# leepaul009/LaneGCN-1

Measured on AMD Instinct MI355X. Metric: Argoverse scenes/sec forward (batch=32, ~10k lane nodes), higher is better.
Workload: dtype f32 (2 fp16 planes per operand, 3 products, fp32 accumulate; range-guarded); 1 GPU; S2: hot path forward (graph_gather+CSR plan+MapNet+A2M+M2M+M2A+A2A), 32 scenes/GPU, 10368 lane nodes, 110592 edges, 1600 actors, random-init weights, inputs resident in HBM, hipGraph replay, 4 forwards in flight on 4 streams; scenes_per_gpu=32, parallelism=dp1 (independent scene shards)

## Files before the change

include/lgcn.h:

```cpp
#ifndef LGCN_H
#define LGCN_H

#include <stdint.h>

#ifdef __cplusplus
extern "C" {
#endif

#define LGCN_VERSION 100
#define LGCN_C 128
#define LGCN_TM 16
#define LGCN_MAX_REL 16

enum {
    LGCN_OK = 0,
    LGCN_EINVAL = -1,
    LGCN_ESHAPE = -2,
    LGCN_EALIGN = -3
};

int lgcn_version(void);
const char *lgcn_strerror(int code);


int lgcn_graph_gather(const int64_t *in, int64_t n_elem,
                      const int64_t *seg_off, const int64_t *seg_base, int n_seg,
                      int64_t *out64, int32_t *out32, void *stream);

int64_t lgcn_csr_rowptr_elems(int64_t n_nodes, int n_rel);
int64_t lgcn_csr_ws_elems(int64_t n_nodes, int n_rel);
int lgcn_csr_build(const int64_t *const *u_host, const int64_t *const *v_host,
                   const int64_t *n_edges_host, int n_rel, int64_t n_nodes,
                   int32_t *rowptr, int32_t *col, int32_t *ws, void *stream);

int64_t lgcn_pairs_ws_elems(int64_t n_agt, int n_scenes);
int lgcn_pairs_build(const float *agt_ctrs, const int32_t *agt_off,
                     const float *ctx_ctrs, const int32_t *ctx_off,
                     int n_scenes, int64_t n_agt, int64_t n_ctx,
                     float dist_th, int legacy_offsets,
                     int32_t *hi, int32_t *wi, int64_t cap,
                     int32_t *n_pairs, int32_t *rowptr, int32_t *ws,
                     void *stream);

typedef struct {
    const float *agt_ctrs; const int32_t *agt_off;
    const float *ctx_ctrs; const int32_t *ctx_off;
    int32_t n_scenes; int32_t legacy_offsets;
    int64_t n_agt, n_ctx;
    float dist_th; int32_t pad_;
    int32_t *hi, *wi; int64_t cap;
    int32_t *n_pairs, *rowptr, *ws;
} lgcn_pairs_job_t;
int lgcn_pairs_build_multi(const lgcn_pairs_job_t *jobs, int n_jobs, void *stream);

typedef struct {
    const int64_t *idx_local; int64_t n_elem;
    const int64_t *seg_off, *seg_base; int32_t n_seg, n_rel;
    int64_t u_off[LGCN_MAX_REL], v_off[LGCN_MAX_REL], n_edges[LGCN_MAX_REL];
    int64_t n_nodes;
    int32_t *rowptr, *col;
    void *cnt;
    int32_t *uv;
    const lgcn_pairs_job_t *jobs; int32_t n_jobs, pad_;
    int32_t *clear_word;
} lgcn_index_t;
int64_t lgcn_index_uv_elems(int64_t n_edges);
int64_t lgcn_index_cnt_words(int64_t n_nodes, int n_rel);
int lgcn_index_build(const lgcn_index_t *p_host, void *stream);


int64_t lgcn_conv_packed_bytes(int cin, int cout, int ks);
int lgcn_conv_pack_weight(const float *w, int cin, int cout, int ks, void *out, void *stream);
int lgcn_conv1d_gn(const float *x, int64_t n_act, int lin, int cin, const void *wp, int cout, int ks, int stride,
                   const float *gamma, const float *beta, float eps, const float *res, int res_mode, int relu,
                   float *out, void *stream);

int lgcn_conv1d_gn_train(const float *x, int64_t n_act, int lin, int cin, const void *wp, int cout, int ks, int stride,
                         const float *gamma, const float *beta, float eps, const float *res, int res_mode, int relu,
                         float *out, float *y, void *stream);

int64_t lgcn_conv_packed_t_bytes(int cin, int cout, int ks);
int lgcn_conv_pack_weight_t(const float *w, int cin, int cout, int ks, void *out, void *stream);
int64_t lgcn_conv1d_gn_bwd_ws_bytes(int64_t n_act, int lin, int cin, int cout, int ks, int stride);
int lgcn_conv1d_gn_bwd(const float *g, const float *x, const float *y, const float *out, int64_t n_act, int lin, int cin,
                       const void *wt, int cout, int ks, int stride, const float *gamma, float eps, int res_mode, int relu,
                       float *dx, float *dw, float *dgamma, float *dbeta, float *dres, void *ws, void *stream);

int lgcn_res1d_gn(const float *x, int64_t n_act, int lin, int cin, int c, int stride, const void *w1p, const float *g1,
                  const float *b1, const void *w2p, const float *g2, const float *b2, const void *wdp, const float *gd,
                  const float *bd, float eps, float *out, void *stream);
int lgcn_res1d_pair_gn(const float *x, int64_t n_act, int lin, int cin, int c, int stride, const void *w1p, const float *g1,
                       const float *b1, const void *w2p, const float *g2, const float *b2, const void *wdp, const float *gd,
                       const float *bd, const void *w1q, const float *g1q, const float *b1q, const void *w2q, const float *g2q,
                       const float *b2q, float eps, float *out, void *stream);


typedef struct lgcn_pred_reg {
    const float *h[8];
    const float *w[8];
    const float *b[8];
    const float *ctrs;
    const float *wd, *bd;
    float *reg, *hd;
    int64_t n_act;
    int32_t n_mod, np2;
} lgcn_pred_reg_t;
int lgcn_pred_reg(const lgcn_pred_reg_t *q, void *stream);

int lgcn_pred_final(const float *f, const float *wc, const float *bc, const float *reg, const float *rot, const float *orig,
                    int64_t n_act, int n_mod, int n_pred, float *cls, float *out, void *stream);

int lgcn_pred_final_train(const float *f, const float *wc, const float *bc, const float *reg, int64_t n_act, int n_mod,
                          int np2, float *cls, float *out, int32_t *order, void *stream);

int64_t lgcn_pred_final_bwd_ws_elems(int64_t n_act);
int lgcn_pred_final_bwd(const float *g_cls, const float *g_out, const int32_t *order, const float *f, const float *wc,
                        int64_t n_act, int n_mod, int np2, float *g_reg, float *d_f, float *d_wc, float *d_bc, float *part,
                        void *stream);

typedef struct lgcn_pred_reg_bwd {
    const float *g_reg;
    const float *g_hd;
    const float *h[8];
    const float *w[8];
    const float *hd, *reg, *ctrs;
    float *d_h[8];
    float *d_w[8];
    float *d_b[8];
    float *d_wd, *d_bd;
    float *part;
    int64_t n_act;
    int32_t n_mod, np2;
} lgcn_pred_reg_bwd_t;
int64_t lgcn_pred_reg_bwd_ws_elems(int64_t n_act, int n_mod, int np2);
int lgcn_pred_reg_bwd(const lgcn_pred_reg_bwd_t *q, void *stream);


int64_t lgcn_scan_ws_elems(int64_t n);
int lgcn_bool_square_bound(const int32_t *rowptr, const int32_t *col, int64_t n, int32_t *cand_ptr, int32_t *ws,
                           void *stream);
int lgcn_bool_square(const int32_t *rowptr, const int32_t *col, int64_t n, const int32_t *cand_ptr, int32_t *cand,
                     int32_t *out_rowptr, int32_t *ws, void *stream);
int lgcn_bool_square_compact(const int32_t *cand_ptr, const int32_t *cand, const int32_t *out_rowptr, int64_t n,
                             int32_t *out_col, int32_t *out_row, void *stream);

int lgcn_cross_edges(const float *ctrs, const float *feats, const int64_t *lane_idcs, int64_t n_nodes, int num_lanes,
                     const int64_t *side_pairs, int64_t n_side, const int64_t *pre_pairs, int64_t n_pre,
                     const int64_t *suc_pairs, int64_t n_suc, float cross_dist, uint8_t *mat, int32_t *partner,
                     void *stream);

int lgcn_widen_i32(const int32_t *in, const int32_t *n_dev, int64_t cap,
// ... 318 lines not shown
```

lanegcn-1_amd/_lib.py:

```python
import ctypes as C
import os

_HERE = os.path.dirname(os.path.abspath(__file__))
LIB_PATH = os.path.join(_HERE, "liblgcn.so")

MAX_REL = 16
REL_IDENT, REL_CSR, REL_RANGE, REL_RANGE16 = 0, 1, 2, 3
F_GN1, F_RELU1, F_GEMM2, F_GN2, F_RES, F_RELU2 = 1, 2, 4, 8, 16, 32
MMA_F32, MMA_BF16X3, MMA_BF16, MMA_F16X2 = 0, 1, 2, 3
MMA_NAMES = {"f32": MMA_F32, "bf16x3": MMA_BF16X3, "bf16": MMA_BF16, "f16x2": MMA_F16X2}


class LgcnError(RuntimeError):
    pass


class Rel(C.Structure):
    _fields_ = [("src", C.c_void_p), ("wp", C.c_void_p), ("mode", C.c_int32), ("ridx", C.c_int32)]


class PairsJob(C.Structure):
    _fields_ = [
        ("agt_ctrs", C.c_void_p), ("agt_off", C.c_void_p), ("ctx_ctrs", C.c_void_p), ("ctx_off", C.c_void_p),
        ("n_scenes", C.c_int32), ("legacy_offsets", C.c_int32), ("n_agt", C.c_int64), ("n_ctx", C.c_int64),
        ("dist_th", C.c_float), ("pad_", C.c_int32),
        ("hi", C.c_void_p), ("wi", C.c_void_p), ("cap", C.c_int64),
        ("n_pairs", C.c_void_p), ("rowptr", C.c_void_p), ("ws", C.c_void_p),
    ]


class Index(C.Structure):
    _fields_ = [
        ("idx_local", C.c_void_p), ("n_elem", C.c_int64),
        ("seg_off", C.c_void_p), ("seg_base", C.c_void_p), ("n_seg", C.c_int32), ("n_rel", C.c_int32),
        ("u_off", C.c_int64 * MAX_REL), ("v_off", C.c_int64 * MAX_REL), ("n_edges", C.c_int64 * MAX_REL),
        ("n_nodes", C.c_int64),
        ("rowptr", C.c_void_p), ("col", C.c_void_p), ("cnt", C.c_void_p), ("uv", C.c_void_p),
        ("jobs", C.c_void_p), ("n_jobs", C.c_int32), ("pad_", C.c_int32),
        ("clear_word", C.c_void_p),
    ]


class PredReg(C.Structure):
    _fields_ = [
        ("h", C.c_void_p * 8), ("w", C.c_void_p * 8), ("b", C.c_void_p * 8),
        ("ctrs", C.c_void_p), ("wd", C.c_void_p), ("bd", C.c_void_p), ("reg", C.c_void_p), ("hd", C.c_void_p),
        ("n_act", C.c_int64), ("n_mod", C.c_int32), ("np2", C.c_int32),
    ]


class PredRegBwd(C.Structure):
    _fields_ = [
        ("g_reg", C.c_void_p), ("g_hd", C.c_void_p), ("h", C.c_void_p * 8), ("w", C.c_void_p * 8),
        ("hd", C.c_void_p), ("reg", C.c_void_p), ("ctrs", C.c_void_p),
        ("d_h", C.c_void_p * 8), ("d_w", C.c_void_p * 8), ("d_b", C.c_void_p * 8),
        ("d_wd", C.c_void_p), ("d_bd", C.c_void_p), ("part", C.c_void_p),
        ("n_act", C.c_int64), ("n_mod", C.c_int32), ("np2", C.c_int32),
    ]


class AttPairsBwd(C.Structure):
    _fields_ = [
        ("agt_ctrs", C.c_void_p), ("ctx_ctrs", C.c_void_p), ("hi", C.c_void_p), ("wi", C.c_void_p), ("n_pairs", C.c_void_p),
        ("cap", C.c_int64),
        ("wd0", C.c_void_p), ("bd0", C.c_void_p), ("wpd2", C.c_void_p), ("gd", C.c_void_p), ("btd", C.c_void_p),
        ("wpc0e", C.c_void_p), ("U", C.c_void_p), ("V", C.c_void_p), ("gc", C.c_void_p), ("btc", C.c_void_p),
        ("wptd2", C.c_void_p), ("wptc0e", C.c_void_p), ("masks", C.c_void_p), ("dS", C.c_void_p),
        ("dc", C.c_void_p), ("d_wd2", C.c_void_p), ("d_wc0e", C.c_void_p), ("d_wd0", C.c_void_p), ("d_bd0", C.c_void_p),
        ("d_gd", C.c_void_p), ("d_btd", C.c_void_p), ("d_gc", C.c_void_p), ("d_btc", C.c_void_p), ("ws", C.c_void_p),
        ("eps", C.c_float), ("n_chunks", C.c_int32),
    ]


class PoolPairsBwd(C.Structure):
    _fields_ = [
        ("ctx_pose", C.c_void_p), ("tgt_pose", C.c_void_p), ("ti", C.c_void_p), ("ci", C.c_void_p), ("n_pairs", C.c_void_p),
        ("cap", C.c_int64),
        ("wp", C.c_void_p), ("bp", C.c_void_p), ("wpc0h", C.c_void_p), ("U", C.c_void_p), ("g", C.c_void_p), ("bt", C.c_void_p),
        ("wptc0h", C.c_void_p), ("masks", C.c_void_p), ("dS", C.c_void_p),
        ("dz", C.c_void_p), ("d_w0h", C.c_void_p), ("d_wp", C.c_void_p), ("d_bp", C.c_void_p), ("d_g", C.c_void_p),
        ("d_bt", C.c_void_p), ("ws", C.c_void_p),
        ("eps", C.c_float), ("n_chunks", C.c_int32),
    ]


class LaneConvBwd(C.Structure):
    _fields_ = [
        ("d_out", C.c_void_p), ("out", C.c_void_p), ("Z", C.c_void_p), ("Y", C.c_void_p), ("T", C.c_void_p), ("X", C.c_void_p),
        ("gamma1", C.c_void_p), ("gamma2", C.c_void_p), ("wpt2", C.c_void_p), ("wpt1", C.c_void_p),
        ("dT", C.c_void_p), ("g2", C.c_void_p), ("dX", C.c_void_p),
        ("d_w2", C.c_void_p), ("d_w1", C.c_void_p), ("d_g2", C.c_void_p), ("d_b2", C.c_void_p), ("d_g1", C.c_void_p),
        ("d_b1", C.c_void_p), ("ws", C.c_void_p),
        ("n_rows", C.c_int64), ("eps", C.c_float), ("n_chunks", C.c_int32), ("ident1", C.c_int32), ("pad_", C.c_int32),
    ]


class RowBlockBwd(C.Structure):
    _fields_ = [
        ("d_out", C.c_void_p), ("out", C.c_void_p), ("pre", C.c_void_p), ("gamma", C.c_void_p),
        ("src", C.c_void_p * 2), ("wpt", C.c_void_p * 2), ("d_src", C.c_void_p * 2), ("d_w", C.c_void_p * 2),
        ("d_res", C.c_void_p), ("d_gamma", C.c_void_p), ("d_beta", C.c_void_p), ("ws", C.c_void_p),
        ("n_rows", C.c_int64), ("ld_w", C.c_int32 * 2), ("eps", C.c_float), ("n_rel", C.c_int32), ("n_chunks", C.c_int32),
        ("pad_", C.c_int32),
    ]


class AggMlp(C.Structure):
    _fields_ = [
        ("n_rows", C.c_int64), ("n_rel", C.c_int32), ("n_rel_csr", C.c_int32),
        ("flags", C.c_int32), ("eps", C.c_float), ("mma", C.c_int32), ("tile_rb", C.c_int32),
        ("rel", Rel * MAX_REL),
        ("rowptr", C.c_void_p), ("col", C.c_void_p),
        ("x4_a", C.c_void_p), ("x4_b", C.c_void_p), ("x4_c", C.c_void_p), ("w4", C.c_void_p),
        ("gn1_g", C.c_void_p), ("gn1_b", C.c_void_p),
        ("wp2", C.c_void_p), ("gn2_g", C.c_void_p), ("gn2_b", C.c_void_p),
        ("res", C.c_void_p), ("out", C.c_void_p), ("out_pre", C.c_void_p),
        ("out_mid", C.c_void_p), ("out_pre2", C.c_void_p),
        ("ch_wq", C.c_void_p), ("ch_gq_g", C.c_void_p), ("ch_gq_b", C.c_void_p), ("ch_wu", C.c_void_p),
        ("ch_u_out", C.c_void_p), ("ch_wv", C.c_void_p), ("ch_v_out", C.c_void_p),
    ]


# ... 30 lines not shown
        ("agent_nodes", C.c_void_p), ("agent_vel", C.c_void_p),
        ("roi_agent", C.c_void_p), ("roi_base", C.c_void_p),
        ("node_mask", C.c_void_p), ("out_feats", C.c_void_p), ("agent_feat", C.c_void_p), ("near", C.c_void_p),
        ("edge_cnt", C.c_void_p),
        ("edge_base", C.c_void_p), ("out_u", C.c_void_p), ("out_v", C.c_void_p), ("a2m_v", C.c_void_p),
    ]


OPT_ADAM, OPT_ADAMW, OPT_SGD = 0, 1, 2
OPT_KINDS = {"adam": OPT_ADAM, "adamw": OPT_ADAMW, "sgd": OPT_SGD}

_P, _I, _L, _F, _D = C.c_void_p, C.c_int, C.c_int64, C.c_float, C.c_double

SIGNATURES = {
    "lgcn_version": (C.c_int, []),
    "lgcn_strerror": (C.c_char_p, [_I]),
    "lgcn_graph_gather": (C.c_int, [_P, _L, _P, _P, _I, _P, _P, _P]),
    "lgcn_csr_rowptr_elems": (C.c_int64, [_L, _I]),
    "lgcn_csr_ws_elems": (C.c_int64, [_L, _I]),
    "lgcn_csr_build": (C.c_int, [_P, _P, _P, _I, _L, _P, _P, _P, _P]),
    "lgcn_pairs_ws_elems": (C.c_int64, [_L, _I]),
    "lgcn_pairs_build": (C.c_int, [_P, _P, _P, _P, _I, _L, _L, _F, _I, _P, _P, _L, _P, _P, _P, _P]),
    "lgcn_pairs_build_multi": (C.c_int, [_P, _I, _P]),
    "lgcn_widen_i32": (C.c_int, [_P, _P, _L, _P, _P]),
    "lgcn_packed_bytes": (C.c_int64, [_I, _I]),
    "lgcn_pack_weight": (C.c_int, [_P, _I, _I, _I, _I, _P, _P]),
    "lgcn_pack_weight_t": (C.c_int, [_P, _I, _I, _P, _P]),
    "lgcn_pack_weight_batch": (C.c_int, [_P, _I, _I, _P]),
    "lgcn_agg_mlp": (C.c_int, [C.POINTER(AggMlp), _P]),
    "lgcn_lc_config": (C.c_int, [_I, _I, C.POINTER(C.c_int32), C.POINTER(C.c_int32)]),
    "lgcn_lc_plan_elems": (C.c_int64, [_L, _I, _I]),
    "lgcn_lc_part_elems": (C.c_int64, [_L, _I, _I]),
    "lgcn_lc_plan_build": (C.c_int, [_P, _P, _L, _I, _I, _I, _I, C.POINTER(C.c_int32), _P, _P]),
    "lgcn_laneconv_fwd": (C.c_int, [C.POINTER(LaneConv), _P]),
    "lgcn_agg_mlp_pair": (C.c_int, [C.POINTER(AggMlp), C.POINTER(AggMlp), _P]),
    "lgcn_agg_mlp_multi": (C.c_int, [C.POINTER(C.POINTER(AggMlp)), _I, _P]),
    "lgcn_gn_bwd": (C.c_int, [_P, _P, _P, _P, _L, _F, _P, _P, _P, _P, _P, _P]),
    "lgcn_gn_fwd": (C.c_int, [_P, _P, _P, _P, _L, _F, _I, _P, _P]),
    "lgcn_gn_cl": (C.c_int, [_P, _L, _I, _I, _P, _P, _F, _P, _I, _I, _I, _P, _P]),
    "lgcn_gn_cl_bwd": (C.c_int, [_P, _P, _P, _P, _L, _I, _I, _F, _P, _P, _P, _P]),
    "lgcn_wgrad": (C.c_int, [C.POINTER(AggMlp), _P, _P, _P, _I, _P]),
    "lgcn_gather_rows": (C.c_int, [_P, _P, _P, _L, _P, _P]),
    "lgcn_gather_sum": (C.c_int, [_P, _P, _P, _L, _P, _P]),
    "lgcn_pair_add": (C.c_int, [_P, _P, _P, _P, _P, _P, _L, _P, _P]),
    "lgcn_check_finite": (C.c_int, [_P, _L, _P, _L, _P, _I, _P]),
    "lgcn_mapnet_input": (C.c_int, [_P, _P, _L] + [_P] * 10 + [_F, _I, _P, _P]),
    "lgcn_att_pairs": (C.c_int, [_P, _P, _P, _P, _P, _L] + [_P] * 10 + [_F, _I, _P, _P]),
    "lgcn_att_pairs_train": (C.c_int, [_P, _P, _P, _P, _P, _L] + [_P] * 10 + [_F, _P, _P, _P]),
    "lgcn_pool_pairs": (C.c_int, [_P, _P, _P, _P, _P, _L] + [_P] * 6 + [_F, _P, _P]),
    "lgcn_pool_pairs_train": (C.c_int, [_P, _P, _P, _P, _P, _L] + [_P] * 6 + [_F, _P, _P, _P]),
    "lgcn_pool_pairs_bwd_ws_elems": (C.c_int64, [_L, _I]),
    "lgcn_pool_pairs_bwd": (C.c_int, [C.POINTER(PoolPairsBwd), _P]),
    "lgcn_att_pairs_bwd_ws_elems": (C.c_int64, [_L, _I]),
    "lgcn_att_pairs_bwd": (C.c_int, [C.POINTER(AttPairsBwd), _P]),
    "lgcn_laneconv_bwd_ws_elems": (C.c_int64, [_L, _I, _I]),
    "lgcn_laneconv_bwd": (C.c_int, [C.POINTER(LaneConvBwd), _P]),
    "lgcn_rowblock_bwd_ws_elems": (C.c_int64, [_L, _I, _I]),
    "lgcn_rowblock_bwd": (C.c_int, [C.POINTER(RowBlockBwd), _P]),
    "lgcn_conv_packed_bytes": (C.c_int64, [_I, _I, _I]),
    "lgcn_conv_pack_weight": (C.c_int, [_P, _I, _I, _I, _P, _P]),
    "lgcn_conv1d_gn": (C.c_int, [_P, _L, _I, _I, _P, _I, _I, _I, _P, _P, _F, _P, _I, _I, _P, _P]),
    "lgcn_conv1d_gn_train": (C.c_int, [_P, _L, _I, _I, _P, _I, _I, _I, _P, _P, _F, _P, _I, _I, _P, _P, _P]),
    "lgcn_conv_packed_t_bytes": (C.c_int64, [_I, _I, _I]),
    "lgcn_conv_pack_weight_t": (C.c_int, [_P, _I, _I, _I, _P, _P]),
    "lgcn_conv1d_gn_bwd_ws_bytes": (C.c_int64, [_L, _I, _I, _I, _I, _I]),
    "lgcn_conv1d_gn_bwd": (C.c_int, [_P, _P, _P, _P, _L, _I, _I, _P, _I, _I, _I, _P, _F, _I, _I, _P, _P, _P, _P, _P, _P, _P]),
    "lgcn_res1d_gn": (C.c_int, [_P, _L, _I, _I, _I, _I, _P, _P, _P, _P, _P, _P, _P, _P, _P, _F, _P, _P]),
    "lgcn_res1d_pair_gn": (C.c_int, [_P, _L, _I, _I, _I, _I, _P, _P, _P, _P, _P, _P, _P, _P, _P, _P, _P, _P, _P, _P, _P, _F, _P, _P]),
    "lgcn_pred_reg": (C.c_int, [C.POINTER(PredReg), _P]),
    "lgcn_pred_final": (C.c_int, [_P, _P, _P, _P, _P, _P, _L, _I, _I, _P, _P, _P]),
    "lgcn_pred_final_train": (C.c_int, [_P, _P, _P, _P, _L, _I, _I, _P, _P, _P, _P]),
    "lgcn_pred_final_bwd_ws_elems": (C.c_int64, [_L]),
    "lgcn_pred_final_bwd": (C.c_int, [_P, _P, _P, _P, _P, _L, _I, _I, _P, _P, _P, _P, _P, _P]),
    "lgcn_pred_reg_bwd_ws_elems": (C.c_int64, [_L, _I, _I]),
    "lgcn_pred_reg_bwd": (C.c_int, [C.POINTER(PredRegBwd), _P]),
    "lgcn_scan_ws_elems": (C.c_int64, [_L]),
    "lgcn_bool_square_bound": (C.c_int, [_P, _P, _L, _P, _P, _P]),
    "lgcn_bool_square": (C.c_int, [_P, _P, _L, _P, _P, _P, _P, _P]),
    "lgcn_bool_square_compact": (C.c_int, [_P, _P, _P, _L, _P, _P, _P]),
    "lgcn_cross_edges": (C.c_int, [_P, _P, _P, _L, _I, _P, _L, _P, _L, _P, _L, _F, _P, _P, _P]),
    "lgcn_index_uv_elems": (C.c_int64, [_L]),
    "lgcn_index_cnt_words": (C.c_int64, [_L, _I]),
    "lgcn_index_build": (C.c_int, [_P, _P]),
    "lgcn_att_pairs_ws": (C.c_int, [_P, _P, _P, _P, _P, _L] + [_P] * 10 + [_F, _I, _I, _P, _P]),
    "lgcn_att_pairs_wi": (C.c_int, [_P, _P, _P, _P, _P, _L] + [_P] * 10 + [_F, _I, _I, _P, _P]),
    "lgcn_pack_weight_kperm": (C.c_int, [_P, _I, _I, _P, _P]),
    "lgcn_pred_loss_fwd": (C.c_int, [_P, _P, _P, _P, _L, _I, _I, _F, _F, _F, _F, _F, _P, _P, _P, _P]),
    "lgcn_pred_loss_bwd": (C.c_int, [_P, _P, _P, _P, _L, _I, _I, _F, _F, _P, _P, _P, _P, _P, _P]),
    "lgcn_conv_packed_f32_bytes": (C.c_int64, [_I, _I, _I]),
    "lgcn_conv_pack_weight_f32": (C.c_int, [_P, _I, _I, _I, _P, _P]),
    "lgcn_conv1d_gn_f32": (C.c_int, [_P, _L, _I, _I, _P, _I, _I, _I, _P, _P, _F, _P, _I, _I, _P, _P, _P]),
    "lgcn_opt_chunk_elems": (C.c_int, []),
    "lgcn_opt_step": (C.c_int, [_P, _I, _P, _I, _I, _D, _D, _D, _D, _D, _D, _I, _D, _D, _I, _F, _F, _P]),
    "lgcn_nms_select": (C.c_int, [_P, _P, _P, _L, _I, _F, _I, _I, _P, _P, _P]),
    "lgcn_goal_decode": (C.c_int, [_P, _P, _P, _L, _P, _P, _L, _P, _P, _P, _P, _P, _I, _I, _F, _P, _P, _P, _P, _P, _P]),
    "lgcn_goal_refine": (C.c_int, [_P, _P, _P, _L, _P, _P]),
    "lgcn_goal_refine_bwd": (C.c_int, [_P, _P, _P, _P, _L, _P, _P, _P, _P]),
    "lgcn_goal_decode_bwd": (C.c_int, [_P, _P, _P, _L, _P, _P, _L, _P, _P, _P, _P, _P, _I, _I, _P, _P, _P, _P, _P, _P, _P]),
    "lgcn_roi_loss_fwd": (C.c_int, [_P, _P, _P, _P, _P, _L, _I, _I, _F, _P, _P, _P, _P, _P]),
    "lgcn_roi_loss_bwd": (C.c_int, [_P, _P, _P, _P, _P, _L, _I, _I, _F, _P, _P, _P, _P, _P, _P, _P, _P]),
    "lgcn_roi_max_lanes": (C.c_int, []),
    "lgcn_roi_max_levels": (C.c_int, []),
    "lgcn_roi_ws_elems": (C.c_int64, [_L, _L, _L, _L, _L]),
    "lgcn_roi_search": (C.c_int, [C.POINTER(Roi), _P]),
    "lgcn_roi_nodes": (C.c_int, [C.POINTER(Roi), _P]),
    "lgcn_roi_edge_count": (C.c_int, [C.POINTER(Roi), _P]),
    "lgcn_roi_edge_fill": (C.c_int, [C.POINTER(Roi), _P]),
}

_lib = None


def load():
    global _lib
    if _lib is not None:
        return _lib
    if not os.path.exists(LIB_PATH):
        raise LgcnError(
            "liblgcn.so not found at %s -- the HIP extension is required (no CPU fallback). "
            "Build it with `python -c 'import __graft_entry__ as g; g.build()'` or "
            "`make -C lanegcn-1_amd/csrc`." % LIB_PATH
        )
    lib = C.CDLL(LIB_PATH)
    for name, (res, args) in SIGNATURES.items():
        fn = getattr(lib, name)
        fn.restype = res
        fn.argtypes = args
    _lib = lib
    return lib


def check(rc, what):
    if rc != 0:
        msg = load().lgcn_strerror(int(rc)).decode()
        raise LgcnError("%s failed: %s (code %d)" % (what, msg, rc))
```

lanegcn-1_amd/csrc/lgcn_index.hip:

```cpp
#include "lgcn_common.hpp"

namespace lgcn {

constexpr int kScanThreads = 256;
constexpr int kScanItems = 8;
constexpr int kScanTile = kScanThreads * kScanItems;

template <int CTRL, int ROW_MASK>
__device__ __forceinline__ int dpp_add_from(int v) {
    return v + __builtin_amdgcn_update_dpp(0, v, CTRL, ROW_MASK, 0xf, false);
}
__device__ __forceinline__ int wave_inclusive_scan(int v, int ) {
    v = dpp_add_from<0x111, 0xf>(v);
    v = dpp_add_from<0x112, 0xf>(v);
    v = dpp_add_from<0x114, 0xf>(v);
    v = dpp_add_from<0x118, 0xf>(v);
    v = dpp_add_from<0x142, 0xa>(v);
    v = dpp_add_from<0x143, 0xc>(v);
    return v;
}

template <int NT>
__device__ __forceinline__ int block_exclusive_scan(int v, int *total, int *lds ) {
    const int lane = threadIdx.x & 63, w = threadIdx.x >> 6;
    const int inc = wave_inclusive_scan(v, lane);
    if (lane == 63) lds[w] = inc;
    __syncthreads();
    if (w == 0) {
        const int t = lane < NT / 64 ? lds[lane] : 0;
        const int run = wave_inclusive_scan(t, lane);
        if (lane < NT / 64) lds[lane] = run - t;
        if (lane == NT / 64 - 1) lds[NT / 64] = run;
    }
    __syncthreads();
    const int base = lds[w];
    *total = lds[NT / 64];
    __syncthreads();
    return base + inc - v;
}

__global__ __launch_bounds__(kScanThreads) void k_scan_blocks(const int32_t *in, int32_t *out,
                                                              int32_t *sums, int64_t n) {
    __shared__ int lds[kScanThreads / 64 + 1];
    const int64_t base = (int64_t)blockIdx.x * kScanTile + (int64_t)threadIdx.x * kScanItems;
    int v[kScanItems];
    int s = 0;
#pragma unroll
    for (int i = 0; i < kScanItems; ++i) {
        v[i] = (base + i < n) ? in[base + i] : 0;
        s += v[i];
    }
    int total;
    int pre = block_exclusive_scan<kScanThreads>(s, &total, lds);
#pragma unroll
    for (int i = 0; i < kScanItems; ++i) {
        if (base + i < n) out[base + i] = pre;
        pre += v[i];
    }
    if (threadIdx.x == 0) sums[blockIdx.x] = total;
}

__global__ __launch_bounds__(1024) void k_scan_sums(int32_t *sums, int nb) {
    __shared__ int lds[1024 / 64 + 1];
    int carry = 0;
    for (int c = 0; c < nb; c += 1024) {
        const int i = c + threadIdx.x;
        const int v = i < nb ? sums[i] : 0;
        int total;
        const int pre = block_exclusive_scan<1024>(v, &total, lds);
        if (i < nb) sums[i] = pre + carry;
        carry += total;
    }
}

__global__ __launch_bounds__(kScanThreads) void k_scan_add_prefix(int32_t *out, const int32_t *sums, int64_t n) {
    __shared__ int lds[kScanThreads / 64 + 1];
    int part = 0;
    for (int i = threadIdx.x; i < (int)blockIdx.x; i += kScanThreads) part += sums[i];
    int add;
    block_exclusive_scan<kScanThreads>(part, &add, lds);
    const int64_t base = (int64_t)blockIdx.x * kScanTile + (int64_t)threadIdx.x * kScanItems;
#pragma unroll
    for (int i = 0; i < kScanItems; ++i)
// ... 170 lines not shown
    __device__ int32_t *wi_base() const { return ws + (n_agt + 1) + n_scenes + 1; }
};
struct PairsJobs { PairsJob j[4]; };

template <int PASS>
__global__ __launch_bounds__(256) void k_pairs_rows(const PairsJobs jobs) {
    const PairsJob &j = jobs.j[blockIdx.y];
    pairs_rows_body<PASS>(j.agt, j.agt_off, j.ctx, j.ctx_off, j.n_scenes, j.n_agt, j.n_ctx, j.th, j.rp(), j.rp(), j.hi_base(),
                          j.wi_base(), j.hi, j.wi, j.cap, j.legacy, j.rowptr_q, (int)blockIdx.x);
}

__device__ __forceinline__ void pairs_scan_bases_body(int32_t *rp, int n_agt, const int32_t *agt_off,
                                                      const int32_t *ctx_off, int n_scenes, int legacy, int64_t cap,
                                                      int32_t *hi_base, int32_t *wi_base, int32_t *n_pairs) {
    __shared__ int lds[1024 / 64 + 1];
    int tot = 0;
    for (int64_t c0 = 0; c0 <= n_agt; c0 += 4096) {
        const int64_t b = c0 + 4 * (int64_t)threadIdx.x;
        int v[4], sum = 0;
#pragma unroll
        for (int k = 0; k < 4; ++k) {
            v[k] = b + k < n_agt ? rp[b + k] : 0;
            sum += v[k];
        }
        int chunk;
        int off = block_exclusive_scan<1024>(sum, &chunk, lds) + tot;
#pragma unroll
        for (int k = 0; k < 4; ++k) {
            if (b + k <= n_agt) rp[b + k] = off;
            off += v[k];
        }
        tot += chunk;
    }
    __syncthreads();
    int carry_h = 0, carry_w = 0;
    for (int c = 0; c < n_scenes; c += 1024) {
        const int i = c + threadIdx.x;
        int th = 0, tw = 0;
        if (i < n_scenes) {
            int a0 = agt_off[i], a1 = agt_off[i + 1];
            a0 = a0 < 0 ? 0 : a0 > n_agt ? n_agt : a0;
            a1 = a1 < a0 ? a0 : a1 > n_agt ? n_agt : a1;
            const bool nonempty = rp[a1] - rp[a0] > 0;
            if (!legacy || nonempty) { th = a1 - a0; tw = ctx_off[i + 1] - ctx_off[i]; }
        }
        int tot_h, tot_w;
        const int ph = block_exclusive_scan<1024>(th, &tot_h, lds);
        const int pw = block_exclusive_scan<1024>(tw, &tot_w, lds);
        if (i < n_scenes) { hi_base[i] = ph + carry_h; wi_base[i] = pw + carry_w; }
        carry_h += tot_h;
        carry_w += tot_w;
    }
    if (threadIdx.x == 0) {
        hi_base[n_scenes] = carry_h;
        *n_pairs = (int64_t)tot > cap ? -tot : tot;
    }
}

__global__ __launch_bounds__(1024) void k_pairs_scan_bases(const PairsJobs jobs) {
    const PairsJob &j = jobs.j[blockIdx.x];
    pairs_scan_bases_body(j.rp(), j.n_agt, j.agt_off, j.ctx_off, j.n_scenes, j.legacy, j.cap, j.hi_base(), j.wi_base(),
                          j.n_pairs);
    if (j.n_agt == 0 && threadIdx.x == 0) j.rowptr_q[0] = 0;
}

constexpr int kIdxScanTile = 4096;
constexpr int kIdxMaxTiles = 1024;

struct IndexParams {
    const int64_t *idx_local, *seg_off, *seg_base;
    int n_seg, n_rel;
    int64_t u_off[LGCN_MAX_REL], v_off[LGCN_MAX_REL];
    int64_t start[LGCN_MAX_REL + 1];
    int64_t n_nodes, n_keys1;
    unsigned long long *cnt;
    int32_t *uv;
    int32_t *rowptr, *col;
    int edge_blocks, scan_blocks, n_jobs;
    int job_blocks[5];
    int32_t *clear_word;
    PairsJobs jobs;
};

__device__ __forceinline__ int64_t to_global(const IndexParams &p, int64_t i) {
    int lo = 0, hi = p.n_seg;
    while (hi - lo > 1) {
        const int mid = (lo + hi) >> 1;
        if (p.seg_off[mid] <= i) lo = mid; else hi = mid;
    }
    return p.idx_local[i] + p.seg_base[lo];
}

template <int PASS>
__global__ __launch_bounds__(256) void k_index_edges(const IndexParams p) {
    __shared__ int s_tile[kIdxMaxTiles];
    const int bid = blockIdx.x;
    if (PASS == 0 && bid == 0 && threadIdx.x == 0 && p.clear_word) *p.clear_word = 0;
    if (bid >= p.edge_blocks) {
        const int b = bid - p.edge_blocks;
        int jn = 0;
        while (jn + 1 < p.n_jobs && b >= p.job_blocks[jn + 1]) ++jn;
        const PairsJob &j = p.jobs.j[jn];
        pairs_rows_body<PASS>(j.agt, j.agt_off, j.ctx, j.ctx_off, j.n_scenes, j.n_agt, j.n_ctx, j.th, j.rp(), j.rp(), j.hi_base(),
                              j.wi_base(), j.hi, j.wi, j.cap, j.legacy, j.rowptr_q, b - p.job_blocks[jn]);
        return;
    }
    if (PASS == 0) {
        for (int i = threadIdx.x; i < p.scan_blocks; i += blockDim.x) s_tile[i] = 0;
        __syncthreads();
    }
    const int64_t total = p.start[p.n_rel];
    for (int64_t e = (int64_t)bid * blockDim.x + threadIdx.x; e < total; e += (int64_t)p.edge_blocks * blockDim.x) {
        int r = 0;
        while (r + 1 < p.n_rel && e >= p.start[r + 1]) ++r;
        if (PASS == 0) {
            const int64_t le = e - p.start[r];
            const int64_t u = to_global(p, p.u_off[r] + le), v = to_global(p, p.v_off[r] + le);
            const bool ok = u >= 0 && u < p.n_nodes && v >= 0 && v < p.n_nodes;
            p.uv[2 * e] = ok ? (int32_t)u : -1;
            p.uv[2 * e + 1] = (int32_t)v;
            if (ok) {
                const int64_t k = csr_key(u, r, p.n_rel);
                atomicAdd(&p.cnt[k], 1ull);
                atomicAdd(&s_tile[k / kIdxScanTile], 1);
            }
        } else {
            const int u = p.uv[2 * e], v = p.uv[2 * e + 1];
            if (u < 0) continue;
            const int64_t k = csr_key(u, r, p.n_rel);
            const unsigned long long a = atomicAdd(&p.cnt[k], 1ull << 32);
            p.col[p.rowptr[k] + (int)(a >> 32)] = v;
        }
    }
    if (PASS == 0) {
        __syncthreads();
        for (int i = threadIdx.x; i < p.scan_blocks; i += blockDim.x)
            if (s_tile[i] != 0) atomicAdd(&p.cnt[p.n_keys1 + i], (unsigned long long)s_tile[i]);
    }
}

__global__ __launch_bounds__(1024) void k_index_scan(const IndexParams p) {
    __shared__ int lds[1024 / 64 + 1];
    const int bid = blockIdx.x;
    if (bid >= p.scan_blocks) {
        const PairsJob &j = p.jobs.j[bid - p.scan_blocks];
        pairs_scan_bases_body(j.rp(), j.n_agt, j.agt_off, j.ctx_off, j.n_scenes, j.legacy, j.cap, j.hi_base(), j.wi_base(),
                              j.n_pairs);
        if (j.n_agt == 0 && threadIdx.x == 0) j.rowptr_q[0] = 0;
        return;
    }
    const int part = (int)threadIdx.x < bid ? (int)p.cnt[p.n_keys1 + threadIdx.x] : 0;
    int before;
    block_exclusive_scan<1024>(part, &before, lds);
    const int64_t b = (int64_t)bid * kIdxScanTile + 4 * (int64_t)threadIdx.x;
    int v[4], sum = 0;
#pragma unroll
    for (int k = 0; k < 4; ++k) {
        v[k] = b + k < p.n_keys1 ? (int)(p.cnt[b + k] & 0xffffffffull) : 0;
        sum += v[k];
    }
    int tile_total;
    int off = block_exclusive_scan<1024>(sum, &tile_total, lds) + before;
#pragma unroll
    for (int k = 0; k < 4; ++k) {
        if (b + k < p.n_keys1) p.rowptr[b + k] = off;
        off += v[k];
    }
}

__global__ __launch_bounds__(256) void k_index_sort(const IndexParams p) {
    const int64_t k = (int64_t)blockIdx.x * blockDim.x + threadIdx.x;
    if (k < kIdxMaxTiles) p.cnt[p.n_keys1 + k] = 0ull;
    if (k >= p.n_keys1) return;
    const unsigned long long w = p.cnt[k];
    if (w == 0ull) return;
    p.cnt[k] = 0ull;
    const int n = (int)(w & 0xffffffffull);
    int32_t *c = p.col + p.rowptr[k];
    for (int i = 1; i < n; ++i) {
        const int x = c[i];
        int q = i - 1;
        while (q >= 0 && c[q] > x) { c[q + 1] = c[q]; --q; }
        c[q + 1] = x;
    }
}

__global__ __launch_bounds__(256) void k_sq_bound(const int32_t *rowptr, const int32_t *col, int64_t n, int32_t *ub) {
    const int64_t u = (int64_t)blockIdx.x * blockDim.x + threadIdx.x;
    if (u > n) return;
    int s = 0;
    if (u < n)
        for (int e = rowptr[u]; e < rowptr[u + 1]; ++e) {
            const int v = col[e];
            if (v >= 0 && v < n) s += rowptr[v + 1] - rowptr[v];
        }
    ub[u] = s;
}

__global__ __launch_bounds__(256) void k_sq_expand(const int32_t *rowptr, const int32_t *col, int64_t n,
                                                   const int32_t *cand_ptr, int32_t *cand, int32_t *cnt) {
    const int64_t u = (int64_t)blockIdx.x * blockDim.x + threadIdx.x;
    if (u > n) return;
    if (u == n) { cnt[n] = 0; return; }
    int32_t *c = cand + cand_ptr[u];
    int k = 0;
    for (int e = rowptr[u]; e < rowptr[u + 1]; ++e) {
        const int v = col[e];
        if (v < 0 || v >= n) continue;
        for (int f = rowptr[v]; f < rowptr[v + 1]; ++f) {
            const int w = col[f];
            int q = k - 1;
            while (q >= 0 && c[q] > w) --q;
            if (q >= 0 && c[q] == w) continue;
            for (int r = k; r > q + 1; --r) c[r] = c[r - 1];
            c[q + 1] = w;
            ++k;
        }
    }
    cnt[u] = k;
}

__global__ __launch_bounds__(256) void k_sq_compact(const int32_t *cand_ptr, const int32_t *cand, const int32_t *out_rowptr,
                                                    int64_t n, int32_t *out_col, int32_t *out_row) {
    const int64_t u = (int64_t)blockIdx.x * blockDim.x + threadIdx.x;
    if (u >= n) return;
    const int b = out_rowptr[u], k = out_rowptr[u + 1] - b;
    const int32_t *c = cand + cand_ptr[u];
    for (int i = 0; i < k; ++i) {
        out_col[b + i] = c[i];
        if (out_row) out_row[b + i] = (int32_t)u;
    }
}

__global__ __launch_bounds__(256) void k_lane_mask(const int64_t *side, int64_t n_side, const int64_t *pre, int64_t n_pre,
                                                   const int64_t *suc, int64_t n_suc, int num_lanes, uint8_t *mat) {
    const int64_t per = n_pre + n_suc + 1;
    const int64_t t = (int64_t)blockIdx.x * blockDim.x + threadIdx.x;
    if (t >= n_side * per) return;
    const int64_t i = t / per, j = t % per;
    const int64_t a = side[2 * i], c = side[2 * i + 1];
    if (a < 0 || a >= num_lanes || c < 0 || c >= num_lanes) return;
    int64_t b = c;
    if (j > 0) {
        const int64_t *pp = j - 1 < n_pre ? pre + 2 * (j - 1) : suc + 2 * (j - 1 - n_pre);
        if (pp[0] != c) return;
        b = pp[1];
        if (b < 0 || b >= num_lanes) return;
    }
    mat[a * num_lanes + b] = 1;
}

__global__ __launch_bounds__(256) void k_cross_edges(const float2 *ctrs, const float2 *feats, const int64_t *lane_idcs,
                                                     int n, const uint8_t *mat, int num_lanes, float cross_dist,
                                                     int32_t *partner) {
    const int lane = threadIdx.x & 63;
    const int h = blockIdx.x * (blockDim.x >> 6) + (threadIdx.x >> 6);
    if (h >= n) return;
    const float2 a = ctrs[h];
    const int64_t la = lane_idcs[h];
    const bool la_ok = la >= 0 && la < num_lanes;
    float best = 3.0e38f;
    int bw = 0x7fffffff;
    for (int w0 = 0; w0 < n; w0 += 64) {
        const int w = w0 + lane;
        if (w < n) {
            const int64_t lb = lane_idcs[w];
            const bool ok = la_ok && lb >= 0 && lb < num_lanes && mat[la * num_lanes + lb] != 0;
// ... 103 lines not shown
        t.v[r] = v_host[r];
        t.start[r + 1] = t.start[r] + n_edges_host[r];
    }
    for (int r = n_rel; r < LGCN_MAX_REL; ++r) { t.u[r] = nullptr; t.v[r] = nullptr; t.start[r + 1] = t.start[n_rel]; }
    const int64_t total = t.start[n_rel];
    if (total > 0x7fffffff || n_nodes > 0x7fffffff) return LGCN_ESHAPE;
    if (total > 0) LGCN_CHECK_PTR(col);
    const int64_t nk1 = lgcn_csr_rowptr_elems(n_nodes, n_rel);
    int32_t *cursor = ws;
    int32_t *sums = ws + nk1;
    hipLaunchKernelGGL(k_zero2, dim3(grid_for(nk1, 256, 1024)), dim3(256), 0, st, rowptr, cursor, nk1);
    if (total > 0) {
        hipLaunchKernelGGL((k_csr_edges<0>), dim3(grid_for(total, 256)), dim3(256), 0, st, t, rowptr, nullptr, nullptr);
    }
    int rc = exclusive_scan(rowptr, rowptr, nk1, sums, st);
    if (rc != LGCN_OK) return rc;
    if (total > 0) {
        hipLaunchKernelGGL((k_csr_edges<1>), dim3(grid_for(total, 256)), dim3(256), 0, st, t, cursor, rowptr, col);
        hipLaunchKernelGGL(k_csr_sort_rows, dim3((unsigned)((nk1 - 1 + 255) / 256)), dim3(256), 0, st,
                           rowptr, col, nk1 - 1);
    }
    return launch_status();
}

int64_t lgcn_pairs_ws_elems(int64_t n_agt, int n_scenes) {
    if (n_agt < 0 || n_scenes < 0) return LGCN_EINVAL;
    return (n_agt + 1) + 2 * (int64_t)n_scenes + 1;
}

static int pairs_job_check(const lgcn_pairs_job_t &q) {
    if (q.n_scenes < 1 || q.n_agt < 0 || q.n_ctx < 0 || q.cap < 0) return LGCN_EINVAL;
    if (q.n_agt > 0x7ffffff0 || q.n_ctx > 0x7ffffff0 || q.cap > 0x7ffffff0) return LGCN_ESHAPE;
    LGCN_CHECK_PTR(q.agt_off); LGCN_CHECK_PTR(q.ctx_off); LGCN_CHECK_PTR(q.n_pairs);
    LGCN_CHECK_PTR(q.rowptr); LGCN_CHECK_PTR(q.ws);
    if (q.n_agt > 0) LGCN_CHECK_PTR(q.agt_ctrs);
    if (q.n_ctx > 0) LGCN_CHECK_PTR(q.ctx_ctrs);
    if (q.cap > 0) { LGCN_CHECK_PTR(q.hi); LGCN_CHECK_PTR(q.wi); }
    return LGCN_OK;
}

int lgcn_pairs_build_multi(const lgcn_pairs_job_t *jobs, int n_jobs, void *stream) {
    if (n_jobs < 1 || n_jobs > 4) return LGCN_EINVAL;
    LGCN_CHECK_PTR(jobs);
    hipStream_t st = (hipStream_t)stream;
    PairsJobs dj;
    int64_t max_rows = 0;
    for (int k = 0; k < n_jobs; ++k) {
        const lgcn_pairs_job_t &q = jobs[k];
        const int rc = pairs_job_check(q);
        if (rc != LGCN_OK) return rc;
        PairsJob &d = dj.j[k];
        d.agt = (const float2 *)q.agt_ctrs; d.agt_off = q.agt_off;
        d.ctx = (const float2 *)q.ctx_ctrs; d.ctx_off = q.ctx_off;
        d.n_scenes = q.n_scenes; d.n_agt = (int)q.n_agt; d.n_ctx = (int)q.n_ctx; d.legacy = q.legacy_offsets; d.th = q.dist_th;
        d.hi = q.hi; d.wi = q.wi; d.cap = q.cap; d.n_pairs = q.n_pairs; d.rowptr_q = q.rowptr; d.ws = q.ws;
        if (q.n_agt > max_rows) max_rows = q.n_agt;
    }
    for (int k = n_jobs; k < 4; ++k) dj.j[k] = dj.j[0];
    const unsigned row_blocks = (unsigned)((max_rows + 3) / 4);
    if (max_rows > 0) hipLaunchKernelGGL((k_pairs_rows<0>), dim3(row_blocks, n_jobs), dim3(256), 0, st, dj);
    hipLaunchKernelGGL(k_pairs_scan_bases, dim3(n_jobs), dim3(1024), 0, st, dj);
    if (max_rows > 0) hipLaunchKernelGGL((k_pairs_rows<1>), dim3(row_blocks, n_jobs), dim3(256), 0, st, dj);
    return launch_status();
}

int lgcn_pairs_build(const float *agt_ctrs, const int32_t *agt_off, const float *ctx_ctrs,
                     const int32_t *ctx_off, int n_scenes, int64_t n_agt, int64_t n_ctx, float dist_th,
                     int legacy_offsets, int32_t *hi, int32_t *wi, int64_t cap, int32_t *n_pairs,
                     int32_t *rowptr, int32_t *ws, void *stream) {
    lgcn_pairs_job_t q;
    q.agt_ctrs = agt_ctrs; q.agt_off = agt_off; q.ctx_ctrs = ctx_ctrs; q.ctx_off = ctx_off;
    q.n_scenes = n_scenes; q.legacy_offsets = legacy_offsets; q.n_agt = n_agt; q.n_ctx = n_ctx;
    q.dist_th = dist_th; q.pad_ = 0; q.hi = hi; q.wi = wi; q.cap = cap; q.n_pairs = n_pairs; q.rowptr = rowptr; q.ws = ws;
    return lgcn_pairs_build_multi(&q, 1, stream);
}

int64_t lgcn_index_uv_elems(int64_t n_edges) { return n_edges < 0 ? (int64_t)LGCN_EINVAL : 2 * n_edges; }

int64_t lgcn_index_cnt_words(int64_t n_nodes, int n_rel) {
    const int64_t k = lgcn_csr_rowptr_elems(n_nodes, n_rel);
    return k < 0 ? k : k + kIdxMaxTiles;
}

int lgcn_index_build(const lgcn_index_t *ph, void *stream) {
    LGCN_CHECK_PTR(ph);
    const lgcn_index_t &q = *ph;
    if (q.n_rel < 1 || q.n_rel > LGCN_MAX_REL || q.n_nodes < 0 || q.n_seg < 1 || q.n_jobs < 0 || q.n_jobs > 4 || q.n_elem < 0)
        return LGCN_EINVAL;
    LGCN_CHECK_PTR(q.rowptr); LGCN_CHECK_PTR(q.cnt);
    if (((uintptr_t)q.cnt & 7u) != 0) return LGCN_EALIGN;
    if (q.n_jobs > 0) LGCN_CHECK_PTR(q.jobs);
    IndexParams p;
    p.idx_local = q.idx_local; p.seg_off = q.seg_off; p.seg_base = q.seg_base; p.n_seg = q.n_seg; p.n_rel = q.n_rel;
    p.start[0] = 0;
    for (int r = 0; r < q.n_rel; ++r) {
        if (q.n_edges[r] < 0 || q.u_off[r] < 0 || q.v_off[r] < 0 || q.u_off[r] + q.n_edges[r] > q.n_elem ||
            q.v_off[r] + q.n_edges[r] > q.n_elem)
            return LGCN_EINVAL;
        p.u_off[r] = q.u_off[r]; p.v_off[r] = q.v_off[r];
        p.start[r + 1] = p.start[r] + q.n_edges[r];
    }
    for (int r = q.n_rel; r < LGCN_MAX_REL; ++r) { p.u_off[r] = p.v_off[r] = 0; p.start[r + 1] = p.start[q.n_rel]; }
    const int64_t total = p.start[q.n_rel];
    if (total > 0x7fffffff || q.n_nodes > 0x7fffffff) return LGCN_ESHAPE;
    const int64_t nk1 = lgcn_csr_rowptr_elems(q.n_nodes, q.n_rel);
    if (nk1 > (int64_t)kIdxScanTile * kIdxMaxTiles) return LGCN_ESHAPE;
    if (total > 0) {
        LGCN_CHECK_PTR(q.idx_local); LGCN_CHECK_PTR(q.seg_off); LGCN_CHECK_PTR(q.seg_base);
        LGCN_CHECK_PTR(q.col); LGCN_CHECK_PTR(q.uv);
    }
    p.n_nodes = q.n_nodes; p.n_keys1 = nk1;
    p.cnt = reinterpret_cast<unsigned long long *>(q.cnt); p.uv = q.uv; p.rowptr = q.rowptr; p.col = q.col;
    p.n_jobs = q.n_jobs;
    p.clear_word = q.clear_word;
    p.job_blocks[0] = 0;
    for (int k = 0; k < 4; ++k) {
        if (k < q.n_jobs) {
            const lgcn_pairs_job_t &jq = q.jobs[k];
            const int rc = pairs_job_check(jq);
            if (rc != LGCN_OK) return rc;
            PairsJob &d = p.jobs.j[k];
            d.agt = (const float2 *)jq.agt_ctrs; d.agt_off = jq.agt_off;
            d.ctx = (const float2 *)jq.ctx_ctrs; d.ctx_off = jq.ctx_off;
            d.n_scenes = jq.n_scenes; d.n_agt = (int)jq.n_agt; d.n_ctx = (int)jq.n_ctx; d.legacy = jq.legacy_offsets; d.th = jq.dist_th;
            d.hi = jq.hi; d.wi = jq.wi; d.cap = jq.cap; d.n_pairs = jq.n_pairs; d.rowptr_q = jq.rowptr; d.ws = jq.ws;
            p.job_blocks[k + 1] = p.job_blocks[k] + (int)((jq.n_agt + 3) / 4);
        } else {
            if (k > 0) p.jobs.j[k] = p.jobs.j[0];
            p.job_blocks[k + 1] = p.job_blocks[k];
        }
    }
    if (q.n_jobs == 0) {
        PairsJob z{};
        for (int k = 0; k < 4; ++k) p.jobs.j[k] = z;
    }
    p.edge_blocks = total > 0 ? (int)grid_for(total, 256, 1024) : 0;
    p.scan_blocks = (int)((nk1 + kIdxScanTile - 1) / kIdxScanTile);
    hipStream_t st = (hipStream_t)stream;
    const unsigned g13 = (unsigned)(p.edge_blocks + p.job_blocks[4]);
    if (g13 > 0) hipLaunchKernelGGL((k_index_edges<0>), dim3(g13), dim3(256), 0, st, p);
    else if (q.clear_word) { hipError_t e = hipMemsetAsync(q.clear_word, 0, 4, st); if (e != hipSuccess) return (int)e; }
    hipLaunchKernelGGL(k_index_scan, dim3((unsigned)(p.scan_blocks + q.n_jobs)), dim3(1024), 0, st, p);
    if (g13 > 0) hipLaunchKernelGGL((k_index_edges<1>), dim3(g13), dim3(256), 0, st, p);
    if (total > 0) hipLaunchKernelGGL(k_index_sort, dim3((unsigned)((nk1 + 255) / 256)), dim3(256), 0, st, p);
    return launch_status();
}

int lgcn_bool_square_bound(const int32_t *rowptr, const int32_t *col, int64_t n, int32_t *cand_ptr, int32_t *ws,
                            void *stream) {
    if (n < 0) return LGCN_EINVAL;
    if (n > 0x7ffffff0) return LGCN_ESHAPE;
    LGCN_CHECK_PTR(rowptr); LGCN_CHECK_PTR(cand_ptr); LGCN_CHECK_PTR(ws);
    hipStream_t st = (hipStream_t)stream;
    hipLaunchKernelGGL(k_sq_bound, dim3(grid_for(n + 1, 256, 1 << 22)), dim3(256), 0, st, rowptr, col, n, cand_ptr);
    return exclusive_scan(cand_ptr, cand_ptr, n + 1, ws, st);
}

int lgcn_bool_square(const int32_t *rowptr, const int32_t *col, int64_t n, const int32_t *cand_ptr, int32_t *cand,
                     int32_t *out_rowptr, int32_t *ws, void *stream) {
    if (n < 0) return LGCN_EINVAL;
    if (n > 0x7ffffff0) return LGCN_ESHAPE;
    LGCN_CHECK_PTR(rowptr); LGCN_CHECK_PTR(cand_ptr); LGCN_CHECK_PTR(out_rowptr); LGCN_CHECK_PTR(ws);
    hipStream_t st = (hipStream_t)stream;
    hipLaunchKernelGGL(k_sq_expand, dim3(grid_for(n + 1, 256, 1 << 22)), dim3(256), 0, st, rowptr, col, n, cand_ptr, cand,
                       out_rowptr);
    return exclusive_scan(out_rowptr, out_rowptr, n + 1, ws, st);
}

int lgcn_bool_square_compact(const int32_t *cand_ptr, const int32_t *cand, const int32_t *out_rowptr, int64_t n,
                             int32_t *out_col, int32_t *out_row, void *stream) {
    if (n < 0) return LGCN_EINVAL;
    if (n == 0) return LGCN_OK;
    LGCN_CHECK_PTR(cand_ptr); LGCN_CHECK_PTR(out_rowptr);
    hipLaunchKernelGGL(k_sq_compact, dim3(grid_for(n, 256, 1 << 22)), dim3(256), 0, (hipStream_t)stream, cand_ptr, cand,
                       out_rowptr, n, out_col, out_row);
    return launch_status();
}

int64_t lgcn_scan_ws_elems(int64_t n) { return n < 0 ? (int64_t)LGCN_EINVAL : scan_ws_elems(n); }

int lgcn_cross_edges(const float *ctrs, const float *feats, const int64_t *lane_idcs, int64_t n_nodes, int num_lanes,
                     const int64_t *side_pairs, int64_t n_side, const int64_t *pre_pairs, int64_t n_pre,
                     const int64_t *suc_pairs, int64_t n_suc, float cross_dist, uint8_t *mat, int32_t *partner,
                     void *stream) {
    if (n_nodes < 0 || num_lanes < 0 || n_side < 0 || n_pre < 0 || n_suc < 0) return LGCN_EINVAL;
    if (n_nodes > 0x7ffffff0 || (int64_t)num_lanes * num_lanes > 0x7ffffff0) return LGCN_ESHAPE;
    if (n_nodes == 0) return LGCN_OK;
    LGCN_CHECK_PTR(ctrs); LGCN_CHECK_PTR(feats); LGCN_CHECK_PTR(lane_idcs); LGCN_CHECK_PTR(partner);
    if (num_lanes > 0) LGCN_CHECK_PTR(mat);
    if (n_side > 0) LGCN_CHECK_PTR(side_pairs);
    if (n_pre > 0) LGCN_CHECK_PTR(pre_pairs);
    if (n_suc > 0) LGCN_CHECK_PTR(suc_pairs);
    hipStream_t st = (hipStream_t)stream;
    if (num_lanes > 0) {
        hipError_t e = hipMemsetAsync(mat, 0, (size_t)num_lanes * num_lanes, st);
        if (e != hipSuccess) return (int)e;
    }
    const int64_t work = n_side * (n_pre + n_suc + 1);
    if (work > 0)
        hipLaunchKernelGGL(k_lane_mask, dim3(grid_for(work, 256, 1 << 22)), dim3(256), 0, st, side_pairs, n_side, pre_pairs,
                           n_pre, suc_pairs, n_suc, num_lanes, mat);
    hipLaunchKernelGGL(k_cross_edges, dim3((unsigned)((n_nodes + 3) / 4)), dim3(256), 0, st, (const float2 *)ctrs,
                       (const float2 *)feats, lane_idcs, (int)n_nodes, mat, num_lanes, cross_dist, partner);
    return launch_status();
}

int lgcn_widen_i32(const int32_t *in, const int32_t *n_dev, int64_t cap, int64_t *out, void *stream) {
    if (cap < 0) return LGCN_EINVAL;
    if (cap == 0) return LGCN_OK;
    LGCN_CHECK_PTR(in); LGCN_CHECK_PTR(n_dev); LGCN_CHECK_PTR(out);
    hipLaunchKernelGGL(k_widen, dim3(grid_for(cap, 256, 1024)), dim3(256), 0, (hipStream_t)stream, in, n_dev, cap, out);
    return launch_status();
}

}
```

lanegcn-1_amd/csrc/lgcn_mma_bf.hpp:

```cpp
#pragma once
#include "lgcn_common.hpp"
#include "lgcn_tile.hpp"

namespace lgcn {

typedef __bf16 bf16x8 __attribute__((ext_vector_type(8)));
typedef __bf16 bf16x2 __attribute__((ext_vector_type(2)));
typedef _Float16 f16x8 __attribute__((ext_vector_type(8)));
typedef _Float16 f16x2 __attribute__((ext_vector_type(2)));
typedef float f32x2 __attribute__((ext_vector_type(2)));
typedef float f32x4 __attribute__((ext_vector_type(4)));

constexpr int kLDB = kC + 8;

template <int F> struct Fmt;
template <> struct Fmt<0> {
    static constexpr int NP = 3, NPROD = 6;
    static constexpr int PA[6] = {2, 0, 1, 1, 0, 0}, PB[6] = {0, 2, 1, 0, 1, 0};
    static __device__ __forceinline__ uint32_t pack(float a, float b) {
        const f32x2 v = {a, b};
        return __builtin_bit_cast(uint32_t, __builtin_convertvector(v, bf16x2));
    }
    static __device__ __forceinline__ f32x2 unpack(uint32_t u) {
        return f32x2{__builtin_bit_cast(float, u << 16), __builtin_bit_cast(float, u & 0xffff0000u)};
// ... 127 lines not shown
__device__ __forceinline__ void gemm_pass(const uint16_t *__restrict__ A, const uint4 *__restrict__ Bw,
                                          const uint4 *__restrict__ Bw_next, BPair<F> &r, int wave, int lane,
                                          f32x4 (&acc)[RB][2]) {
    const uint16_t *arow = A + (lane & 15) * kLDB + 8 * (lane >> 4);
    load_b<F>(r.b[1], Bw, wave, lane, 1);
    kstep<RB, F>(arow, 0, r.b[0], acc);
    load_b<F>(r.b[0], Bw, wave, lane, 2);
    kstep<RB, F>(arow, 1, r.b[1], acc);
    load_b<F>(r.b[1], Bw, wave, lane, 3);
    kstep<RB, F>(arow, 2, r.b[0], acc);
    if (Bw_next != nullptr) load_b<F>(r.b[0], Bw_next, wave, lane, 0);
    kstep<RB, F>(arow, 3, r.b[1], acc);
}

template <int F>
__device__ __forceinline__ void gemm2_prefetch(BPair<F> &r, const uint4 *__restrict__ Bw, int wave, int lane) {
    load_b<F>(r.b[1], Bw, wave, lane, 1);
}
template <int F>
__device__ __forceinline__ void gemm2_prefetch(BOne<F> &, const uint4 *__restrict__, int, int) {}
template <int RB, int F>
__device__ __forceinline__ void gemm2_pass(const uint16_t *__restrict__ A, const uint4 *__restrict__ Bw, BOne<F> &r,
                                           int wave, int lane, f32x4 (&acc)[RB][2]) {
    gemm_pass<RB, F>(A, Bw, nullptr, r, wave, lane, acc);
}
template <int RB, int F>
__device__ __forceinline__ void gemm2_pass(const uint16_t *__restrict__ A, const uint4 *__restrict__ Bw, BPair<F> &r,
                                           int wave, int lane, f32x4 (&acc)[RB][2]) {
    const uint16_t *arow = A + (lane & 15) * kLDB + 8 * (lane >> 4);
    kstep<RB, F>(arow, 0, r.b[0], acc);
    load_b<F>(r.b[0], Bw, wave, lane, 2);
    kstep<RB, F>(arow, 1, r.b[1], acc);
    load_b<F>(r.b[1], Bw, wave, lane, 3);
    kstep<RB, F>(arow, 2, r.b[0], acc);
    kstep<RB, F>(arow, 3, r.b[1], acc);
}

template <int RB>
__device__ __forceinline__ void acc_store(float *T, const f32x4 (&acc)[RB][2], int lane, int wave) {
#pragma unroll
    for (int rb = 0; rb < RB; ++rb)
#pragma unroll
        for (int cb = 0; cb < 2; ++cb) {
            float *p = T + (16 * rb + 4 * (lane >> 4)) * kLDA + 32 * wave + 16 * cb + (lane & 15);
#pragma unroll
            for (int i = 0; i < 4; ++i) p[i * kLDA] = acc[rb][cb][i];
        }
}

template <int RB>
__device__ __forceinline__ void acc_zero(f32x4 (&acc)[RB][2]) {
#pragma unroll
    for (int rb = 0; rb < RB; ++rb)
#pragma unroll
        for (int cb = 0; cb < 2; ++cb) acc[rb][cb] = f32x4{0.f, 0.f, 0.f, 0.f};
}

template <int F>
__device__ __forceinline__ void row_split_store(uint16_t *planes, int plane_elems, int row, int t, const RowVals &r) {
#pragma unroll
    for (int j = 0; j < 4; ++j) split_store<F>(planes, plane_elems, row, 4 * (t & 7) + 32 * j, r.v[j]);
}

template <int F>
__device__ __forceinline__ void lin2_relu_split(uint16_t *planes, int plane_elems, int row, int t, float x, float y,
                                                const float *__restrict__ w1, const float *__restrict__ b1) {
    const int c0 = 4 * (t & 7);
#pragma unroll
    for (int j = 0; j < 4; ++j) {
        const int c = c0 + 32 * j;
        const float4 wa = *reinterpret_cast<const float4 *>(w1 + 2 * c);
        const float4 wb = *reinterpret_cast<const float4 *>(w1 + 2 * c + 4);
        const float4 bb = *reinterpret_cast<const float4 *>(b1 + c);
        float4 o;
        o.x = relu_nan(x * wa.x + y * wa.y + bb.x);
        o.y = relu_nan(x * wa.z + y * wa.w + bb.y);
        o.z = relu_nan(x * wb.x + y * wb.y + bb.z);
        o.w = relu_nan(x * wb.z + y * wb.w + bb.w);
        split_store<F>(planes, plane_elems, row, c, o);
    }
}


}
```

lanegcn-1_amd/csrc/lgcn_rowmlp_bf.hip:

```cpp
#include "lgcn_common.hpp"
#include "lgcn_tile.hpp"
#include "lgcn_mma_bf.hpp"
#include <type_traits>

namespace lgcn {

constexpr int LGCN_RB_ONE = 3;

template <int F>
__device__ __forceinline__ void pack_block_bf(const float *__restrict__ W, int ld, uint16_t *__restrict__ out, int transpose,
                                              int i) {
    if (i >= 4 * 4 * 2 * 64) return;
    const int lane = i & 63, cb = (i >> 6) & 1, s = (i >> 7) & 3, w = i >> 9;
    const int orow = 32 * w + 16 * cb + (lane & 15), k0 = 32 * s + 8 * (lane >> 4);
    float v[8];
#pragma unroll
    for (int j = 0; j < 8; ++j) v[j] = transpose ? W[(int64_t)(k0 + j) * ld + orow] : W[(int64_t)orow * ld + k0 + j];
#pragma unroll
    for (int p = 0; p < Fmt<F>::NP; ++p) {
        uint32_t q[4];
#pragma unroll
        for (int j = 0; j < 4; ++j) {
            q[j] = Fmt<F>::pack(v[2 * j], v[2 * j + 1]);
            const f32x2 r = Fmt<F>::unpack(q[j]);
// ... 376 lines not shown
        }
        lds_barrier();
        if (my_live) row_store_global(p.ch_u_out + my_n * kC, my_rt, row_load(T + (upper ? 32 : 0) * kLDA, my_rt));
    };
    if (two && upper) gemm2_prefetch<F>(bfrag, reinterpret_cast<const uint4 *>(p.wp2), wave, lane);
    if (my_has_row) {
        {
            const float *rbase = (flags & LGCN_F_RES) ? p.res : p.out;
            const float *rp_ = rbase + (my_live ? my_n : 0) * kC + 4 * (my_rt & 7);
#pragma unroll
            for (int j = 0; j < 4; ++j) resv.v[j] = *reinterpret_cast<const float4 *>(rp_ + 32 * j);
        }
        RowVals r = row_load(T + (upper ? 32 : 0) * kLDA, my_rt);
#ifndef LGCN_STAMPS
        if (my_live && p.out_pre) row_store_global(p.out_pre + my_n * kC, my_rt, r);
#endif
        if (flags & LGCN_F_GN1) row_gn<F == 0>(r, my_rt, gnp, gnp + kC, p.eps);
        if (!two && my_live && (flags & LGCN_F_RES)) row_add(r, resv);
        if (flags & LGCN_F_RELU1) row_relu(r);
        if (two && my_live && p.out_mid) row_store_global(p.out_mid + my_n * kC, my_rt, r);
        if (two) row_split_store<F>(Yp, TL::PLANE, my_row, my_rt, r);
        else if (my_live) row_store_global(p.out + my_n * kC, my_rt, r);
        if (!two && (chain_u || chain_v)) resv = r;
    }
    if (!two) {
        if (chain_u || chain_v) chained(resv);
        return;
    }
    LGCN_STAMP(42);
    lds_barrier();
    LGCN_STAMP(43);
    if (wave < 4) {
        acc_zero<RB>(acc);
        gemm2_pass<RB, F>(Yp, reinterpret_cast<const uint4 *>(p.wp2), bfrag, wave, lane, acc);
        acc_store<RB>(T, acc, lane, wave);
    }
    LGCN_STAMP(44);
    lds_barrier();
    LGCN_STAMP(45);
    if (my_has_row) {
        RowVals r = row_load(T + (upper ? 32 : 0) * kLDA, my_rt);
        if (my_live && p.out_pre2) row_store_global(p.out_pre2 + my_n * kC, my_rt, r);
        if (flags & LGCN_F_GN2) row_gn<F == 0>(r, my_rt, gnp + 2 * kC, gnp + 3 * kC, p.eps);
        if (my_live && (flags & LGCN_F_RES)) row_add(r, resv);
        if (flags & LGCN_F_RELU2) row_relu(r);
        if (my_live) row_store_global(p.out + my_n * kC, my_rt, r);
        resv = r;
    }
    LGCN_STAMP(46);
    if (chain_u || chain_v) chained(resv);
}

#define LGCN_WAVES_PER_SIMD(RB_, F_) __attribute__((amdgpu_waves_per_eu((F_) != 0 && ((RB_) <= 2 || (RB_) == LGCN_RB_ONE) ? 4 : 2)))

template <int RB, int F, int KIND>
__global__ __launch_bounds__(512) LGCN_WAVES_PER_SIMD(RB, F) void k_agg_mlp_bf(const lgcn_agg_mlp_t p, int n_tiles) {
    __shared__ __attribute__((aligned(16))) unsigned char smem[Tile<RB, F>::SMEM + 128 + TileIdx<RB>::INTS * 4 + 6 * kC * 4];
    agg_body<RB, F, KIND>(p, n_tiles, blockIdx.x, smem);
}

template <int RB, int F>
__global__ __launch_bounds__(512) LGCN_WAVES_PER_SIMD(RB, F) void k_agg_mlp_bf2(const lgcn_agg_mlp_t pa, const lgcn_agg_mlp_t pb, int tiles_a,
                                                                                int tiles_b) {
    __shared__ __attribute__((aligned(16))) unsigned char smem[Tile<RB, F>::SMEM + 128 + TileIdx<RB>::INTS * 4 + 6 * kC * 4];
    if ((int)blockIdx.x < tiles_a) agg_body<RB, F, 0>(pa, tiles_a, blockIdx.x, smem);
    else agg_body<RB, F, 0>(pb, tiles_b, blockIdx.x - tiles_a, smem);
}

struct MultiArgs {
    lgcn_agg_mlp_t p[LGCN_MAX_MULTI];
    int tiles[LGCN_MAX_MULTI];
    int n;
};
template <int RB, int F>
__global__ __launch_bounds__(512) LGCN_WAVES_PER_SIMD(RB, F) void k_agg_mlp_bfn(const MultiArgs m) {
    __shared__ __attribute__((aligned(16))) unsigned char smem[Tile<RB, F>::SMEM + 128 + TileIdx<RB>::INTS * 4 + 6 * kC * 4];
    int b = blockIdx.x, i = 0;
    while (i + 1 < m.n && b >= m.tiles[i]) { b -= m.tiles[i]; ++i; }
    agg_body<RB, F, 0>(m.p[i], m.tiles[i], b, smem);
}

template <int RB, int F>
__global__ __launch_bounds__(256) void k_mapnet_input_bf(const InputParams p, int n_tiles) {
    using TL = Tile<RB, F>;
    constexpr int ROWS = TL::ROWS;
    __shared__ __attribute__((aligned(16))) unsigned char smem[TL::ABUF_BYTES + TL::T_BYTES];
    uint16_t *A = reinterpret_cast<uint16_t *>(smem);
    float *T = reinterpret_cast<float *>(smem + TL::ABUF_BYTES);
    const int tid = threadIdx.x, lane = tid & 63, wave = tid >> 6;
    const int64_t row0 = (int64_t)blockIdx.x * ROWS;
    f32x4 acc[RB][2];
    RowVals keep[(ROWS + 31) / 32];

#pragma unroll
    for (int br = 0; br < 2; ++br) {
        const float2 *xy = reinterpret_cast<const float2 *>(br == 0 ? p.ctrs : p.feats);
        const float *w1 = br == 0 ? p.wa1 : p.ws1, *b1 = br == 0 ? p.ba1 : p.bs1;
        const float *wp = br == 0 ? p.wpa2 : p.wps2;
        const float *g = br == 0 ? p.ga : p.gs, *bt = br == 0 ? p.bta : p.bts;
#pragma unroll
        for (int c0 = 0; c0 < ROWS; c0 += 32) {
            const int row = c0 + (tid >> 3);
            if (row < ROWS) {
                float2 v = make_float2(0.f, 0.f);
                if (row0 + row < p.n_rows) v = xy[row0 + row];
                lin2_relu_split<F>(A, TL::PLANE, row, tid, v.x, v.y, w1, b1);
            }
        }
        lds_barrier();
        acc_zero<RB>(acc);
        {
            BPair<F> bf;
            ring_prime<F>(bf, reinterpret_cast<const uint4 *>(wp), wave, lane);
            gemm_pass<RB, F>(A, reinterpret_cast<const uint4 *>(wp), nullptr, bf, wave, lane, acc);
        }
        acc_store<RB>(T, acc, lane, wave);
        lds_barrier();
#pragma unroll
        for (int c0 = 0; c0 < ROWS; c0 += 32) {
            const int row = c0 + (tid >> 3);
            if (row < ROWS) {
                RowVals r = row_load(T + c0 * kLDA, tid);
                row_gn<F == 0>(r, tid, g, bt, p.eps);
                if (br == 0) {
                    keep[c0 / 32] = r;
                } else {
#pragma unroll
                    for (int j = 0; j < 4; ++j) r.v[j] = f4add(r.v[j], keep[c0 / 32].v[j]);
                    row_relu(r);
                    if (row0 + row < p.n_rows) row_store_global(p.out + (row0 + row) * kC, tid, r);
                }
            }
        }
    }
}

static int cu_count() {
    int dev = 0, v = 0;
    if (hipGetDevice(&dev) == hipSuccess &&
        hipDeviceGetAttribute(&v, hipDeviceAttributeMultiprocessorCount, dev) == hipSuccess && v > 0)
        return v;
    return 256;
}

static int pick_rb(int64_t n_rows, int fmt, bool lane_conv = false) {
    const int64_t n_sub = (n_rows + 15) / 16;
    auto slots = [&](int rb) { return (int64_t)cu_count() * (fmt != 0 && (rb <= 2 || rb == LGCN_RB_ONE) ? 2 : 1); };
    auto tiles = [&](int rb) { return (n_sub + rb - 1) / rb; };
    if (lane_conv && LGCN_RB_ONE == 3 && fmt != 0 && tiles(2) > cu_count() && tiles(3) <= slots(3)) return 3;
    int best = 1;
    int64_t best_cost = -1;
    for (int rb = 1; rb <= 4; ++rb) {
        const int64_t cost = ((tiles(rb) + slots(rb) - 1) / slots(rb)) * rb;
        if (best_cost < 0 || cost <= best_cost) { best_cost = cost; best = rb; }
    }
    return best;
}

template <int N> using Int = std::integral_constant<int, N>;

template <class Fn>
static int with_fmt(int mma, Fn fn) {
    switch (fmt_of(mma)) {
        case 0: fn(Int<0>{}); break;
        case 1: fn(Int<1>{}); break;
        default: fn(Int<2>{}); break;
    }
    return launch_status();
}

template <class Fn>
static int with_fmt_rb(int mma, int rb, Fn fn) {
    return with_fmt(mma, [&](auto f) {
        switch (rb) {
            case 1: fn(f, Int<1>{}); break;
            case 2: fn(f, Int<2>{}); break;
            case 3: fn(f, Int<3>{}); break;
            default: fn(f, Int<4>{}); break;
        }
    });
}

int agg_mlp_bf(const lgcn_agg_mlp_t &p, bool lane_conv, hipStream_t st) {
    if (p.tile_rb < 0 || p.tile_rb > 4) return LGCN_EINVAL;
    const int rb = p.tile_rb ? p.tile_rb : pick_rb(p.n_rows, fmt_of(p.mma), lane_conv);
    const int n_tiles = (int)((p.n_rows + 16 * rb - 1) / (16 * rb));
    return with_fmt_rb(p.mma, rb, [&](auto f, auto r) {
        constexpr int F = decltype(f)::value, RB = decltype(r)::value;
        if (lane_conv) hipLaunchKernelGGL((k_agg_mlp_bf<RB, F, 1>), dim3(n_tiles), dim3(512), 0, st, p, n_tiles);
        else hipLaunchKernelGGL((k_agg_mlp_bf<RB, F, 0>), dim3(n_tiles), dim3(512), 0, st, p, n_tiles);
    });
}

int agg_mlp_pair_bf(const lgcn_agg_mlp_t &a, const lgcn_agg_mlp_t &b, hipStream_t st) {
    const int rb = pick_rb(a.n_rows > b.n_rows ? a.n_rows : b.n_rows, fmt_of(a.mma));
    const int rows = 16 * rb;
    const int ta = (int)((a.n_rows + rows - 1) / rows), tb = (int)((b.n_rows + rows - 1) / rows);
    return with_fmt_rb(a.mma, rb, [&](auto f, auto r) {
        hipLaunchKernelGGL((k_agg_mlp_bf2<decltype(r)::value, decltype(f)::value>), dim3(ta + tb), dim3(512), 0, st, a, b, ta, tb);
    });
}

int agg_mlp_multi_bf(const lgcn_agg_mlp_t *const *ps, int n, hipStream_t st) {
    int64_t big = 0;
    for (int i = 0; i < n; ++i) big = ps[i]->n_rows > big ? ps[i]->n_rows : big;
    if (ps[0]->tile_rb < 0 || ps[0]->tile_rb > 4) return LGCN_EINVAL;
    const int rb = ps[0]->tile_rb ? ps[0]->tile_rb : pick_rb(big, fmt_of(ps[0]->mma));
    const int rows = 16 * rb;
    MultiArgs m{};
    m.n = n;
    int total = 0;
    for (int i = 0; i < n; ++i) {
        m.p[i] = *ps[i];
        m.tiles[i] = (int)((ps[i]->n_rows + rows - 1) / rows);
        total += m.tiles[i];
    }
    return with_fmt_rb(ps[0]->mma, rb, [&](auto f, auto r) {
        hipLaunchKernelGGL((k_agg_mlp_bfn<decltype(r)::value, decltype(f)::value>), dim3(total), dim3(512), 0, st, m);
    });
}

int mapnet_input_bf(const InputParams &p, int mma, hipStream_t st) {
    const int rb = pick_rb(p.n_rows, fmt_of(mma));
    const int n_tiles = (int)((p.n_rows + 16 * rb - 1) / (16 * rb));
    return with_fmt_rb(mma, rb, [&](auto f, auto r) {
        hipLaunchKernelGGL((k_mapnet_input_bf<decltype(r)::value, decltype(f)::value>), dim3(n_tiles), dim3(256), 0, st, p, n_tiles);
    });
}

int pack_weight_bf(const float *W, int ld, int mma, int transpose, void *out, hipStream_t st) {
    uint16_t *o = reinterpret_cast<uint16_t *>(out);
    return with_fmt(mma, [&](auto f) {
        hipLaunchKernelGGL((k_pack_weight_bf<decltype(f)::value>), dim3(8), dim3(256), 0, st, W, ld, o, transpose);
    });
}

int pack_weight_batch_bf(const lgcn_pack_job_t *jobs, int n_jobs, int mma, hipStream_t st) {
    return with_fmt(mma, [&](auto f) {
        hipLaunchKernelGGL((k_pack_weight_batch_bf<decltype(f)::value>), dim3(8, n_jobs), dim3(256), 0, st, jobs);
    });
}

}
```

lanegcn-1_amd/csrc/lgcn_tile.hpp:

```cpp
#pragma once
#include "lgcn_common.hpp"

namespace lgcn {

struct RowVals { float4 v[4]; };

__device__ __forceinline__ RowVals row_load(const float *T, int t) {
    RowVals r;
    const float *p = T + (t >> 3) * kLDA + 4 * (t & 7);
#pragma unroll
    for (int j = 0; j < 4; ++j) r.v[j] = *reinterpret_cast<const float4 *>(p + 32 * j);
    return r;
}

__device__ __forceinline__ void row_store_lds(float *T, int t, const RowVals &r) {
    float *p = T + (t >> 3) * kLDA + 4 * (t & 7);
#pragma unroll
    for (int j = 0; j < 4; ++j) *reinterpret_cast<float4 *>(p + 32 * j) = r.v[j];
}

template <int CTRL>
__device__ __forceinline__ float dpp_mov(float x) {
    return __builtin_bit_cast(float, __builtin_amdgcn_update_dpp(0, __builtin_bit_cast(int, x), CTRL, 0xf, 0xf, true));
}
// ... 109 lines not shown
        r.v[j].z = relu_nan(r.v[j].z); r.v[j].w = relu_nan(r.v[j].w);
    }
}

__device__ __forceinline__ void row_add_global(RowVals &r, const float *__restrict__ rowp, int t) {
    const float *p = rowp + 4 * (t & 7);
#pragma unroll
    for (int j = 0; j < 4; ++j) {
        const float4 x = *reinterpret_cast<const float4 *>(p + 32 * j);
        r.v[j].x += x.x; r.v[j].y += x.y; r.v[j].z += x.z; r.v[j].w += x.w;
    }
}

__device__ __forceinline__ void row_add(RowVals &r, const RowVals &x) {
#pragma unroll
    for (int j = 0; j < 4; ++j) {
        r.v[j].x += x.v[j].x; r.v[j].y += x.v[j].y; r.v[j].z += x.v[j].z; r.v[j].w += x.v[j].w;
    }
}

__device__ __forceinline__ void row_store_global(float *__restrict__ rowp, int t, const RowVals &r) {
    float *p = rowp + 4 * (t & 7);
#pragma unroll
    for (int j = 0; j < 4; ++j) *reinterpret_cast<float4 *>(p + 32 * j) = r.v[j];
}

__device__ __forceinline__ float4 f4add(float4 a, float4 b) { return make_float4(a.x + b.x, a.y + b.y, a.z + b.z, a.w + b.w); }


struct InputParams {
    const float *ctrs, *feats;
    int64_t n_rows;
    const float *wa1, *ba1, *wpa2, *ga, *bta;
    const float *ws1, *bs1, *wps2, *gs, *bts;
    float eps;
    float *out;
};

struct PairParams {
    const float *agt_ctrs, *ctx_ctrs;
    const int32_t *hi, *wi, *n_pairs;
    int64_t cap;
    const float *wd0, *bd0, *wpd2, *gd, *btd;
    const float *wpc0e, *U, *V, *gc, *btc;
    float eps;
    float *m;
};

struct PoolParams {
    const float *ctx_pose, *tgt_pose;
    const int32_t *ti, *ci, *n_pairs;
    int64_t cap;
    const float *wp, *bp, *wpc0h, *U, *g, *bt;
    float eps;
    float *m;
};

struct PairBwdParams {
    PairParams f;
    const float *wptd2, *wptc0e;
    const uint4 *masks;
    const float *dS;
    float *dc, *rec;
    int want_d, want_wc;
};

struct PairBwdOut { float *dwd2, *dwc0e, *dgc, *dbc, *dgd, *dbd, *dbd0, *dwd0; };

struct PoolBwdParams {
    PoolParams f;
    const float *wptc0h;
    const uint4 *masks;
    const float *dS;
    float *dz, *rec;
    int want_p, want_w;
};

struct PoolBwdOut { float *dw0h, *dwp, *dbp, *dg, *dbt; };

int agg_mlp_bf(const lgcn_agg_mlp_t &p, bool lane_conv, hipStream_t st);
int agg_mlp_pair_bf(const lgcn_agg_mlp_t &a, const lgcn_agg_mlp_t &b, hipStream_t st);
int agg_mlp_multi_bf(const lgcn_agg_mlp_t *const *ps, int n, hipStream_t st);
int mapnet_input_bf(const InputParams &p, int mma, hipStream_t st);
int pack_weight_bf(const float *W, int ld, int mma, int transpose, void *out, hipStream_t st);
int pack_weight_batch_bf(const lgcn_pack_job_t *jobs, int n_jobs, int mma, hipStream_t st);

}
```

lanegcn-1_amd/engine.py:

```python
from dataclasses import dataclass
from typing import Dict, List, Optional

import os

import numpy as np
import torch

from . import ops
from . import lanegcn as M


@dataclass
class FlatBatch:
    n_scenes: int
    n_nodes: int
    n_actors: int
    num_scales: int
    node_ctrs: torch.Tensor
    node_feats: torch.Tensor
    turn: torch.Tensor
    control: torch.Tensor
    intersect: torch.Tensor
    actor_ctrs: torch.Tensor
    node_off: torch.Tensor
    actor_off: torch.Tensor
    idx_local: torch.Tensor
    seg_off: torch.Tensor
    seg_base: torch.Tensor
    rel_slices: List[tuple]
    cap_a2m: int
    cap_a2a: int
    n_edges: List[int]
    _buf: Optional[torch.Tensor] = None

    def buf_view(self) -> Optional[torch.Tensor]:
        return self._buf


_FLAT_ARRAYS = ("node_ctrs", "node_feats", "turn", "control", "intersect", "actor_ctrs", "node_off", "actor_off",
                "idx_local", "seg_off", "seg_base")


@dataclass
class HostFlatBatch:
    buf: torch.Tensor
    layout: Dict[str, tuple]
    meta: Dict

    def to(self, device=None) -> "FlatBatch":
        dev = torch.device("cuda", torch.cuda.current_device()) if device is None else torch.device(device)
        dbuf = self.buf if dev.type == "cpu" else self.buf.to(dev, non_blocking=True)
        arrs = {}
        for name, (off, dt, shape) in self.layout.items():
            cnt = int(np.prod(shape)) if len(shape) else 1
            tdt = {"float32": torch.float32, "int32": torch.int32, "int64": torch.int64}[dt]
            arrs[name] = dbuf[off:off + cnt * np.dtype(dt).itemsize].view(tdt).view(*shape)
        return FlatBatch(**self.meta, **arrs, _buf=dbuf)


def collate_flat_host(scenes: List[Dict], pin: Optional[bool] = None) -> HostFlatBatch:

    def npy(x):
        return x.numpy() if torch.is_tensor(x) else np.asarray(x)

    graphs = [s["graph"] for s in scenes]
    B = len(scenes)
    ns = len(graphs[0]["pre"])
    n_nodes = np.array([int(g["num_nodes"]) for g in graphs], np.int64)
    n_act = np.array([len(s["ctrs"]) for s in scenes], np.int64)
    node_off = np.zeros(B + 1, np.int64)
    np.cumsum(n_nodes, out=node_off[1:])
    actor_off = np.zeros(B + 1, np.int64)
    np.cumsum(n_act, out=actor_off[1:])

    pieces, seg_len, seg_base, rel_slices, n_edges = [], [], [], [], []
    pos = 0

    def add(getter):
        nonlocal pos
        begin = pos
        for j, g in enumerate(graphs):
            x = npy(getter(g)).astype(np.int64, copy=False).reshape(-1)
            pieces.append(x)
            seg_len.append(len(x))
            seg_base.append(node_off[j])
            pos += len(x)
        return (begin, pos)

    keys = []
    for i in range(ns):
        keys += [("pre", i), ("suc", i)]
    for k1, i in keys:
        su = add(lambda g: g[k1][i]["u"])
        sv = add(lambda g: g[k1][i]["v"])
        rel_slices.append((su, sv))
        n_edges.append(su[1] - su[0])
    for k1 in ("left", "right"):
        su = add(lambda g: g[k1]["u"])
        sv = add(lambda g: g[k1]["v"])
        rel_slices.append((su, sv))
        n_edges.append(su[1] - su[0])
    seg_off = np.zeros(len(seg_len) + 1, np.int64)
    np.cumsum(seg_len, out=seg_off[1:])

    cat = lambda key, src: np.concatenate([npy(s[key]) for s in src], 0)
    arrays = {
        "node_ctrs": cat("ctrs", graphs).astype(np.float32, copy=False), "node_feats": cat("feats", graphs).astype(np.float32, copy=False),
        "turn": cat("turn", graphs).astype(np.float32, copy=False), "control": cat("control", graphs).astype(np.float32, copy=False),
        "intersect": cat("intersect", graphs).astype(np.float32, copy=False), "actor_ctrs": cat("ctrs", scenes).astype(np.float32, copy=False),
        "node_off": node_off.astype(np.int32), "actor_off": actor_off.astype(np.int32),
        "idx_local": np.concatenate(pieces) if pieces else np.zeros(0, np.int64),
        "seg_off": seg_off, "seg_base": np.asarray(seg_base, np.int64),
    }
    layout, off = {}, 0
    for name in _FLAT_ARRAYS:
        a = arrays[name]
        layout[name] = (off, str(a.dtype), tuple(a.shape))
        off = (off + a.nbytes + 255) & ~255
    pin = torch.cuda.is_available() if pin is None else pin
    buf = torch.empty(max(off, 256), dtype=torch.uint8, pin_memory=bool(pin))
    view = buf.numpy()
    for name in _FLAT_ARRAYS:
        o, _, _ = layout[name]
        a = np.ascontiguousarray(arrays[name])
        view[o:o + a.nbytes] = a.view(np.uint8).reshape(-1)
    meta = dict(n_scenes=B, n_nodes=int(node_off[-1]), n_actors=int(actor_off[-1]), num_scales=ns,
                rel_slices=rel_slices, cap_a2m=int(np.dot(n_nodes, n_act)), cap_a2a=int(np.dot(n_act, n_act)),
                n_edges=n_edges)
    return HostFlatBatch(buf, layout, meta)


def collate_flat(scenes: List[Dict], device=None, pin: Optional[bool] = None) -> FlatBatch:
    on_cpu = device is not None and torch.device(device).type == "cpu"
    return collate_flat_host(scenes, pin=False if on_cpu else pin).to(device)


def host_actor_inputs(scenes):
    npy = lambda x: x.numpy() if torch.is_tensor(x) else np.asarray(x)
    feats = np.concatenate([npy(s["feats"]).transpose(0, 2, 1) for s in scenes], 0).astype(np.float32)
    rot = np.concatenate([np.repeat(npy(s["rot"])[None], len(s["ctrs"]), 0) for s in scenes]).astype(np.float32)
    orig = np.concatenate([np.repeat(npy(s["orig"])[None], len(s["ctrs"]), 0) for s in scenes]).astype(np.float32)
    t = lambda a: torch.from_numpy(np.ascontiguousarray(a))
    return t(feats), t(rot), t(orig), [len(s["ctrs"]) for s in scenes]


class HotPathEngine:

    def __init__(self, map_net: M.MapNet, a2m: M.A2M, m2m: M.M2M, m2a: M.M2A, a2a: M.A2A, config=None,
                 legacy_offsets: bool = True, branches: bool = False, lane_impl: Optional[str] = None):
        self.map_net, self.a2m, self.m2m, self.m2a, self.a2a = map_net, a2m, m2m, m2a, a2a
        self.config = config or M.config
        self.legacy_offsets = legacy_offsets
        self.lane_impl = lane_impl
        self.branches = branches
        self._side = None
        self._cnt_capture = None
        self.pair_caps = os.environ.get("LGCN_PAIR_CAPS", "tight")
        self._pair_seen = [0, 0, 0]

    def _counters(self, fb: FlatBatch) -> torch.Tensor:
        if self._cnt_capture is not None:
            return self._cnt_capture
        cnt = fb.__dict__.get("_idx_cnt")
        if cnt is None:
            cnt = ops.index_counters(fb.n_nodes, len(fb.rel_slices), fb.node_ctrs.device)
            fb.__dict__["_idx_cnt"] = cnt
        return cnt

    @torch.no_grad()
    def forward(self, fb: FlatBatch, actors: torch.Tensor, stages: bool = False,
                mapnet_only: bool = False) -> Dict[str, torch.Tensor]:
        if mapnet_only:
            g64, _ = ops.graph_gather_indices(fb.idx_local, fb.seg_off, fb.seg_base)
            plan = ops.csr_build([g64[a:b] for (a, b), _ in fb.rel_slices], [g64[a:b] for _, (a, b) in fb.rel_slices],
                                 fb.n_nodes)
            feat = M.lane_conv(self.map_net.fuse, self.map_net.stem(fb.node_ctrs, fb.node_feats), plan, fb.num_scales,
                               impl=self.lane_impl)
            return {"nodes": feat, "actors": actors}
        cfg = self.config
        out = {}
        main = torch.cuda.current_stream()
        side = None
        if self.branches:
            if self._side is None:
                self._side = torch.cuda.Stream()
            side = self._side
        dev = fb.node_ctrs.device
        searches = ((fb.node_ctrs, fb.node_off, fb.actor_ctrs, fb.actor_off, cfg["actor2map_dist"], fb.cap_a2m),
                    (fb.actor_ctrs, fb.actor_off, fb.node_ctrs, fb.node_off, cfg["map2actor_dist"], fb.cap_a2m),
                    (fb.actor_ctrs, fb.actor_off, fb.actor_ctrs, fb.actor_off, cfg["actor2actor_dist"], fb.cap_a2a))
        if self.pair_caps == "tight":
            searches = tuple(s[:5] + (min(s[5], self._cap(i)) if self._pair_seen[i] > 0 else s[5],) for i, s in enumerate(searches))
        bufs = [ops.pairs_alloc(s[0].shape[0], fb.n_scenes, s[5], dev) for s in searches]
        if side is not None:
            side.wait_stream(main)
        if side is None and ops.index_fused_ok(fb.n_nodes, len(fb.rel_slices), sum(fb.n_edges)):
            flag = torch.empty(1, dtype=torch.int32, device=dev)
            plan, pairs = ops.index_build(fb.idx_local, fb.seg_off, fb.seg_base, fb.rel_slices, fb.n_nodes, searches,
                                          self.legacy_offsets, bufs=bufs, cnt=self._counters(fb), clear_word=flag)
        else:
            flag = torch.zeros(1, dtype=torch.int32, device=dev)
            with torch.cuda.stream(side if side is not None else main):
                pairs = ops.pairs_build_multi(searches, self.legacy_offsets, bufs=bufs)
            g64, _ = ops.graph_gather_indices(fb.idx_local, fb.seg_off, fb.seg_base)
            us = [g64[a:b] for (a, b), _ in fb.rel_slices]
            vs = [g64[a:b] for _, (a, b) in fb.rel_slices]
            plan = ops.csr_build(us, vs, fb.n_nodes)
        feat = self.map_net.stem(fb.node_ctrs, fb.node_feats)
        feat = M.lane_conv(self.map_net.fuse, feat, plan, fb.num_scales, impl=self.lane_impl)
        if stages:
            out["map_net"] = feat
        fold = side is None and M._fold_ok(actors) and fb.n_nodes > 0
        if fold:
            feat = self.a2m.run(feat, fb.turn, fb.control, fb.intersect, actors, pairs[0])
        else:
            feat = self.a2m.fuse_meta(feat, fb.turn, fb.control, fb.intersect)
            if side is not None:
                main.wait_stream(side)
            for att in self.a2m.att:
                feat = att.run(feat, actors, pairs[0], side)
        if stages:
            out["a2m"] = feat
        feat = M.lane_conv(self.m2m.fuse, feat, plan, fb.num_scales, impl=self.lane_impl)
        if stages:
            out["m2m"] = feat
        act = actors
        if fold:
            act, uv = M.att_block(self.m2a.att, act, feat, pairs[1], next_att=self.a2a.att[0], next_ctx_is_out=True)
            if stages:
                out["m2a"] = act
            act, _ = M.att_block(self.a2a.att, act, act, pairs[2], uv=uv, ctx_is_agts=True)
        else:
            for att in self.m2a.att:
                act = att.run(act, feat, pairs[1], side)
            if stages:
                out["m2a"] = act
            for att in self.a2a.att:
                act = att.run(act, act, pairs[2], side)
        if stages:
            out["a2a"] = act
        out["nodes"], out["actors"] = feat, act
        out["n_pairs"] = [p.n_pairs for p in pairs]
        ops.check_finite(flag, feat, act)
        out["nonfinite"] = flag
        return out

    def _cap(self, i: int) -> int:
        want = max(4096, int(self._pair_seen[i] * 1.25) + 1)
        return (want + 1023) // 1024 * 1024

    def learn_pair_counts(self, out: Dict[str, torch.Tensor]) -> bool:
        counts = torch.stack([c.view(()) for c in out["n_pairs"]]).tolist()
        over = False
        for i, c in enumerate(counts):
            over = over or c < 0
            self._pair_seen[i] = max(self._pair_seen[i], abs(int(c)))
        return over

    def forward_guarded(self, fb: FlatBatch, actors: torch.Tensor, **kw) -> Dict[str, torch.Tensor]:
        out = self.forward(fb, actors, **kw)
        if self.pair_caps == "tight" and not kw.get("mapnet_only") and self.learn_pair_counts(out):
            out = self.forward(fb, actors, **kw)
            if self.learn_pair_counts(out):
                raise ops.L.LgcnError("pair capacity still exceeded after growing it")
        if ops.get_guard() == "off" or ops.get_mma() != "f16x2" or int(out["nonfinite"].item()) == 0:
            return out
        if ops.get_guard() == "raise":
            raise ops.L.LgcnError("non-finite features in f16x2 mode: an operand left fp16's range (|x| >= 65520)")
        with ops.mma_scope("bf16x3"):
            return self.forward(fb, actors, **kw)

    @torch.no_grad()
    def stage_functions(self, fb: FlatBatch, actors: torch.Tensor):
        cfg, st = self.config, {}

        def index():
            searches = ((fb.node_ctrs, fb.node_off, fb.actor_ctrs, fb.actor_off, cfg["actor2map_dist"], fb.cap_a2m),
                        (fb.actor_ctrs, fb.actor_off, fb.node_ctrs, fb.node_off, cfg["map2actor_dist"], fb.cap_a2m),
                        (fb.actor_ctrs, fb.actor_off, fb.actor_ctrs, fb.actor_off, cfg["actor2actor_dist"], fb.cap_a2a))
            if ops.index_fused_ok(fb.n_nodes, len(fb.rel_slices), sum(fb.n_edges)):
                cnt = st.get("_cnt")
                if cnt is None:
                    cnt = st["_cnt"] = ops.index_counters(fb.n_nodes, len(fb.rel_slices), fb.node_ctrs.device)
                st["plan"], st["pairs"] = ops.index_build(fb.idx_local, fb.seg_off, fb.seg_base, fb.rel_slices, fb.n_nodes,
                                                          searches, self.legacy_offsets, cnt=cnt)
                return
            st["pairs"] = ops.pairs_build_multi(searches, self.legacy_offsets)
            g64, _ = ops.graph_gather_indices(fb.idx_local, fb.seg_off, fb.seg_base)
            st["plan"] = ops.csr_build([g64[a:b] for (a, b), _ in fb.rel_slices],
                                       [g64[a:b] for _, (a, b) in fb.rel_slices], fb.n_nodes)

        def map_net():
            st["nodes"] = M.lane_conv(self.map_net.fuse, self.map_net.stem(fb.node_ctrs, fb.node_feats), st["plan"],
                                      fb.num_scales, impl=self.lane_impl)

        def a2m():
            st["nodes_a2m"] = self.a2m.run(st["nodes"], fb.turn, fb.control, fb.intersect, actors, st["pairs"][0])

        def m2m():
            st["nodes_m2m"] = M.lane_conv(self.m2m.fuse, st["nodes_a2m"], st["plan"], fb.num_scales, impl=self.lane_impl)

        def m2a():
            if M._fold_ok(st["nodes_m2m"]):
                st["actors_m2a"], st["uv_a2a"] = M.att_block(self.m2a.att, actors, st["nodes_m2m"], st["pairs"][1],
                                                             next_att=self.a2a.att[0], next_ctx_is_out=True)
                return
            act = actors
            for att in self.m2a.att:
                act = att.run(act, st["nodes_m2m"], st["pairs"][1])
            st["actors_m2a"], st["uv_a2a"] = act, None

        def a2a():
            act = st["actors_m2a"]
            if M._fold_ok(act):
                st["actors_a2a"] = M.att_block(self.a2a.att, act, act, st["pairs"][2], uv=st["uv_a2a"], ctx_is_agts=True)[0]
                return
            for att in self.a2a.att:
                act = att.run(act, act, st["pairs"][2])
            st["actors_a2a"] = act

        return st, [("index", index), ("map_net", map_net), ("a2m", a2m), ("m2m", m2m), ("m2a", m2a), ("a2a", a2a)]

    def capture(self, fb: FlatBatch, actors: torch.Tensor, warmup: int = 2, **fwd_kw):
        side = torch.cuda.Stream()
        side.wait_stream(torch.cuda.current_stream())
        with torch.cuda.stream(side):
            for _ in range(max(warmup, 2 if self.pair_caps == "tight" else 0)):
                o = self.forward(fb, actors, **fwd_kw)
                if self.pair_caps == "tight" and not fwd_kw.get("mapnet_only"):
                    self.learn_pair_counts(o)
        torch.cuda.current_stream().wait_stream(side)
        torch.cuda.synchronize()
        with self.own_counters(fb) as cnt:
            graph = torch.cuda.CUDAGraph()
            with torch.cuda.graph(graph):
                out = self.forward(fb, actors, **fwd_kw)
        graph._lgcn_inputs = (fb, actors, cnt)
        return graph, out

    def own_counters(self, fb: FlatBatch):
        import contextlib

        @contextlib.contextmanager
        def cm():
            cnt = ops.index_counters(fb.n_nodes, len(fb.rel_slices), fb.node_ctrs.device)
            torch.cuda.synchronize()
            prev, self._cnt_capture = self._cnt_capture, cnt
            try:
                yield cnt
            finally:
                self._cnt_capture = prev
        return cm()


class FullNetEngine:

    def __init__(self, net: "M.Net"):
        self.net = net
        self.hot = HotPathEngine(net.map_net, net.a2m, net.m2m, net.m2a, net.a2a, net.config)

    @staticmethod
    def actor_inputs(scenes, device=None):
        dev = torch.device("cuda", torch.cuda.current_device()) if device is None else torch.device(device)
        feats, rot, orig, _ = host_actor_inputs(scenes)
        return feats.to(dev), rot.to(dev), orig.to(dev)

    @torch.no_grad()
    def forward(self, fb: FlatBatch, actor_feats: torch.Tensor, rot: torch.Tensor, orig: torch.Tensor,
                sizes: List[int], return_pairs: bool = False) -> Dict[str, torch.Tensor]:
        net = self.net
        actors = net.actor_net(actor_feats)
        hot = self.hot.forward(fb, actors)
        actors = hot["actors"]
        if net.pred_net._hip_ok(actors):
            cls, reg = net.pred_net.forward_flat(actors, fb.actor_ctrs, rot, orig)
        else:
            idcs, ctrs, st = [], [], 0
            for n in sizes:
                idcs.append(slice(st, st + n))
                ctrs.append(fb.actor_ctrs[st:st + n])
                st += n
            out = net.pred_net(actors, idcs, ctrs)
            reg = torch.cat(out["reg"], 0)
            cls = torch.cat(out["cls"], 0)
            reg = torch.einsum("amtk,akj->amtj", reg, rot) + orig.view(-1, 1, 1, 2)
        res = {"cls": cls, "reg": reg, "nonfinite": hot["nonfinite"]}
        ops.check_finite(hot["nonfinite"], reg.reshape(-1), cls.reshape(-1), bit=2)
        res["n_pairs"] = hot["n_pairs"]
        return res

    def capture(self, fb, actor_feats, rot, orig, sizes, warmup: int = 3, tune_convs: bool = True,
                capture_error_mode: str = "global", **fwd_kw):
        prev = torch.backends.cudnn.benchmark
        torch.backends.cudnn.benchmark = bool(tune_convs)
        try:
            side = torch.cuda.Stream()
            side.wait_stream(torch.cuda.current_stream())
            with torch.cuda.stream(side):
                for _ in range(warmup):
                    o = self.forward(fb, actor_feats, rot, orig, sizes, **fwd_kw)
                    if self.hot.pair_caps == "tight" and self.hot.learn_pair_counts(o):
                        self.forward(fb, actor_feats, rot, orig, sizes, **fwd_kw)
            torch.cuda.current_stream().wait_stream(side)
            torch.cuda.synchronize()
            with self.hot.own_counters(fb) as cnt:
                graph = torch.cuda.CUDAGraph()
                with torch.cuda.graph(graph, capture_error_mode=capture_error_mode):
                    out = self.forward(fb, actor_feats, rot, orig, sizes, **fwd_kw)
            graph._lgcn_inputs = (fb, actor_feats, rot, orig, cnt)
        finally:
            torch.backends.cudnn.benchmark = prev
        return graph, out
```

lanegcn-1_amd/flatfile.py:

```python
from typing import Dict, List, Sequence

import numpy as np
import torch

from .engine import FlatBatch

_NODE = ("ctrs", "feats", "turn", "control", "intersect")


def _npy(x):
    return x.numpy() if torch.is_tensor(x) else np.asarray(x)


def _relations(graph) -> List[Dict]:
    rels = []
    for i in range(len(graph["pre"])):
        rels += [graph["pre"][i], graph["suc"][i]]
    return rels + [graph["left"], graph["right"]]


def write_scenes(path: str, scenes: Sequence[Dict]) -> None:
    S = len(scenes)
    graphs = [s["graph"] for s in scenes]
    R = 2 * len(graphs[0]["pre"]) + 2
    node_off = np.zeros(S + 1, np.int64)
    np.cumsum([int(g["num_nodes"]) for g in graphs], out=node_off[1:])
    actor_off = np.zeros(S + 1, np.int64)
    np.cumsum([len(s["ctrs"]) for s in scenes], out=actor_off[1:])
    edge_off = np.zeros((R, S + 1), np.int64)
    us, vs = [[] for _ in range(R)], [[] for _ in range(R)]
    for j, g in enumerate(graphs):
        for r, rel in enumerate(_relations(g)):
            u, v = _npy(rel["u"]).reshape(-1), _npy(rel["v"]).reshape(-1)
            us[r].append(u.astype(np.int32))
            vs[r].append(v.astype(np.int32))
            edge_off[r, j + 1] = edge_off[r, j] + len(u)
    rel_off = np.zeros(R + 1, np.int64)
    np.cumsum(edge_off[:, -1], out=rel_off[1:])
    cat = lambda parts, dt: np.concatenate(parts).astype(dt) if parts else np.zeros(0, dt)
    out = dict(
        num_scales=np.int64(len(graphs[0]["pre"])), node_off=node_off, actor_off=actor_off, edge_off=edge_off,
        rel_off=rel_off,
        edge_u=cat([x for r in range(R) for x in us[r]], np.int32), edge_v=cat([x for r in range(R) for x in vs[r]], np.int32),
        actor_ctrs=cat([_npy(s["ctrs"]) for s in scenes], np.float32),
        actor_feats=cat([_npy(s["feats"]) for s in scenes], np.float32),
        rot=np.stack([_npy(s["rot"]) for s in scenes]).astype(np.float32),
        orig=np.stack([_npy(s["orig"]) for s in scenes]).astype(np.float32),
    )
    for k in _NODE:
        out["node_" + k if k in ("ctrs", "feats") else k] = cat([_npy(g[k]) for g in graphs], np.float32)
    if "gt_preds" in scenes[0]:
        out["gt_preds"] = cat([_npy(s["gt_preds"]) for s in scenes], np.float32)
        out["has_preds"] = cat([_npy(s["has_preds"]) for s in scenes], bool)
    np.savez(path, **out)


class FlatSceneFile:

    def __init__(self, path: str):
        with np.load(path, allow_pickle=False) as z:
            self.a = {k: z[k] for k in z.files}
        self.n_scenes = len(self.a["node_off"]) - 1
        self.num_scales = int(self.a["num_scales"])

    def __len__(self):
        return self.n_scenes

    def _rows(self, off, idx):
        return np.concatenate([np.arange(off[i], off[i + 1]) for i in idx]) if len(idx) else np.zeros(0, np.int64)

    def batch(self, indices: Sequence[int], device=None):
        a = self.a
        idx = list(indices)
        dev = torch.device("cuda", torch.cuda.current_device()) if device is None else torch.device(device)
        up = lambda x: torch.from_numpy(np.ascontiguousarray(x)).to(dev)
        n_nodes = np.array([a["node_off"][i + 1] - a["node_off"][i] for i in idx], np.int64)
        n_act = np.array([a["actor_off"][i + 1] - a["actor_off"][i] for i in idx], np.int64)
        node_off = np.zeros(len(idx) + 1, np.int64)
        np.cumsum(n_nodes, out=node_off[1:])
        actor_off = np.zeros(len(idx) + 1, np.int64)
        np.cumsum(n_act, out=actor_off[1:])
        nrow, arow = self._rows(a["node_off"], idx), self._rows(a["actor_off"], idx)
        R = a["edge_off"].shape[0]
        pieces, seg_len, seg_base, rel_slices, n_edges = [], [], [], [], []
        pos = 0
        for r in range(R):
            spans = []
            for which in ("edge_u", "edge_v"):
                begin = pos
                for j, i in enumerate(idx):
                    lo, hi = a["rel_off"][r] + a["edge_off"][r, i], a["rel_off"][r] + a["edge_off"][r, i + 1]
                    pieces.append(a[which][lo:hi].astype(np.int64))
                    seg_len.append(hi - lo)
                    seg_base.append(node_off[j])
                    pos += hi - lo
                spans.append((int(begin), int(pos)))
            rel_slices.append((spans[0], spans[1]))
            n_edges.append(spans[0][1] - spans[0][0])
        seg_off = np.zeros(len(seg_len) + 1, np.int64)
        np.cumsum(seg_len, out=seg_off[1:])
        fb = FlatBatch(
            n_scenes=len(idx), n_nodes=int(node_off[-1]), n_actors=int(actor_off[-1]), num_scales=self.num_scales,
            node_ctrs=up(a["node_ctrs"][nrow]), node_feats=up(a["node_feats"][nrow]), turn=up(a["turn"][nrow]),
            control=up(a["control"][nrow]), intersect=up(a["intersect"][nrow]), actor_ctrs=up(a["actor_ctrs"][arow]),
            node_off=up(node_off.astype(np.int32)), actor_off=up(actor_off.astype(np.int32)),
            idx_local=up(np.concatenate(pieces) if pieces else np.zeros(0, np.int64)), seg_off=up(seg_off),
            seg_base=up(np.asarray(seg_base, np.int64)), rel_slices=rel_slices,
            cap_a2m=int(np.dot(n_nodes, n_act)), cap_a2a=int(np.dot(n_act, n_act)), n_edges=n_edges)
        rep = np.repeat(np.asarray(idx), n_act)
        extras = {"actor_feats": up(a["actor_feats"][arow].transpose(0, 2, 1)), "rot": up(a["rot"][rep]),
                  "orig": up(a["orig"][rep]), "sizes": [int(x) for x in n_act]}
        if "gt_preds" in a:
            extras["gt_preds"], extras["has_preds"] = up(a["gt_preds"][arow]), up(a["has_preds"][arow])
        return fb, extras
```

lanegcn-1_amd/lanegcn.py:

```python
import os
from math import gcd
from typing import Dict, List, Optional

import numpy as np
import torch
from torch import Tensor, nn
from torch.nn import functional as F

from . import _lib as L
from . import autograd as A
from . import ops
from .data import collate_fn
from .layers import Conv1d, Linear, LinearRes, Res1d, group_norm1
from .utils import Optimizer, StepLR, gpu, to_long

file_path = os.path.abspath(__file__)
root_path = os.path.dirname(file_path)
model_name = os.path.basename(file_path).split(".")[0]

config = dict(
    display_iters=205942, val_iters=205942 * 2, save_freq=1.0, epoch=0, horovod=True, opt="adam",
    num_epochs=36, lr=[1e-3, 1e-4], lr_epochs=[32],
    batch_size=32, val_batch_size=32, workers=0, val_workers=0,
    preprocess=True, rot_aug=False, pred_range=[-100.0, 100.0, -100.0, 100.0],
# ... 141 lines not shown
    return plan


def lane_conv_train(fuse: nn.ModuleDict, feat: Tensor, plan: ops.LanePlan, plan_t: ops.LanePlan,
                    num_scales: int, fused_bwd: bool = False) -> Tensor:
    keys = rel_keys(num_scales)
    for i in range(len(fuse["ctr"])):
        rels, weights = [A.Rel(0, 0, L.REL_IDENT)], [fuse["ctr"][i].weight]
        for r, key in enumerate(keys):
            if plan.n_edges[r] > 0:
                rels.append(A.Rel(0, len(weights), L.REL_CSR, r))
                weights.append(fuse[key][i].weight)
        spec = A.BlockSpec(n_rows=feat.shape[0], rels=rels, gn=True, relu=True, has_res=True, eps=fuse["norm"][i].eps,
                           plan=plan, plan_t=plan_t, fused_bwd=fused_bwd)
        c2 = fuse["ctr2"][i]
        feat = A.LaneConvFn.apply(spec, feat, fuse["norm"][i].weight, fuse["norm"][i].bias, c2.linear.weight,
                                  c2.norm.weight, c2.norm.bias, *weights)
    return feat


def _fuse_modules(n_map: int, num_scales: int, ng: int = 1) -> nn.ModuleDict:
    keys = ["ctr", "norm", "ctr2", "left", "right"]
    for i in range(num_scales):
        keys += ["pre%d" % i, "suc%d" % i]
    fuse = {}
    for key in keys:
        if key == "norm":
            mods = [nn.GroupNorm(gcd(ng, n_map), n_map) for _ in range(4)]
        elif key == "ctr2":
            mods = [Linear(n_map, n_map, norm="GN", ng=ng, act=False) for _ in range(4)]
        else:
            mods = [nn.Linear(n_map, n_map, bias=False) for _ in range(4)]
        fuse[key] = nn.ModuleList(mods)
    return nn.ModuleDict(fuse)


def lane_conv(fuse: nn.ModuleDict, feat: Tensor, plan: ops.LanePlan, num_scales: int, tile_rb: int = 0,
              impl: Optional[str] = None) -> Tensor:
    keys = rel_keys(num_scales)
    if impl is None:
        impl = "fused" if ops.get_mma() == "bf16x3" else ops.laneconv_impl()
    lcp = ops.lc_plan(plan) if impl == "tiled" and tile_rb == 0 and plan.n_nodes > 0 else None
    if lcp is not None:
        part = ops.lc_part(lcp)
        for i in range(len(fuse["ctr"])):
            wps = [ops.packed(fuse["ctr"][i].weight)]
            wps += [ops.packed(fuse[key][i].weight) if plan.n_edges[r] > 0 else None for r, key in enumerate(keys)]
            c2 = fuse["ctr2"][i]
            feat = ops.laneconv_fwd(feat, lcp, wps, _gn(fuse["norm"][i]), ops.packed(c2.linear.weight), _gn(c2.norm),
                                    eps=fuse["norm"][i].eps, part=part)
        return feat
    for i in range(len(fuse["ctr"])):
        rels = [ops.RelSpec(feat, ops.packed(fuse["ctr"][i].weight), L.REL_IDENT)]
        for r, key in enumerate(keys):
            if plan.n_edges[r] > 0:
                rels.append(ops.RelSpec(feat, ops.packed(fuse[key][i].weight), L.REL_CSR, r))
        c2 = fuse["ctr2"][i]
        feat = ops.agg_mlp(feat.shape[0], rels, _FULL, rowptr=plan.rowptr, col=plan.col, n_rel_csr=plan.n_rel,
                           gn1=_gn(fuse["norm"][i]), wp2=ops.packed(c2.linear.weight), gn2=_gn(c2.norm),
                           res=feat, eps=fuse["norm"][i].eps, tag="laneconv", tile_rb=tile_rb)
    return feat


class MapNet(nn.Module):
    train_hip = False

    def __init__(self, config):
        super().__init__()
        self.config = config
        n_map = config["n_map"]
        self.input = nn.Sequential(nn.Linear(2, n_map), nn.ReLU(inplace=True),
                                   Linear(n_map, n_map, norm="GN", ng=1, act=False))
        self.seg = nn.Sequential(nn.Linear(2, n_map), nn.ReLU(inplace=True),
                                 Linear(n_map, n_map, norm="GN", ng=1, act=False))
        self.fuse = _fuse_modules(n_map, config["num_scales"])
        self.relu = nn.ReLU(inplace=True)

    def stem(self, ctrs: Tensor, feats: Tensor) -> Tensor:
        a, s = self.input, self.seg
        return ops.mapnet_input(ctrs, feats,
                                a[0].weight, a[0].bias, ops.packed(a[2].linear.weight), _gn(a[2].norm),
                                s[0].weight, s[0].bias, ops.packed(s[2].linear.weight), _gn(s[2].norm),
                                eps=a[2].norm.eps)

    def forward(self, graph):
        if (len(graph["feats"]) == 0 or len(graph["pre"][-1]["u"]) == 0 or len(graph["suc"][-1]["u"]) == 0):
            raise KeyError("node_idcs")
        ctrs = torch.cat(graph["ctrs"], 0)
        if _hot_guard(graph["feats"], *ops.module_params(self)):
            a, s = self.input, self.seg
            fa = A.linear_gn(F.relu(a[0](ctrs)), a[2].linear.weight, gn=a[2].norm)
            fs = A.linear_gn(F.relu(s[0](graph["feats"])), s[2].linear.weight, gn=s[2].norm)
            feat = lane_conv_train(self.fuse, F.relu(fa + fs), lane_plan(graph), lane_plan_t(graph), len(graph["pre"]),
                                   fused_bwd=MapNet.train_hip)
            return feat, graph["idcs"], graph["ctrs"]
        feat = ops.guarded(lambda: lane_conv(self.fuse, self.stem(ctrs, graph["feats"]), lane_plan(graph), len(graph["pre"])))
        return feat, graph["idcs"], graph["ctrs"]


class M2M(nn.Module):
    train_hip = False

    def __init__(self, config):
        super().__init__()
        self.config = config
        self.fuse = _fuse_modules(config["n_map"], config["num_scales"])
        self.relu = nn.ReLU(inplace=True)

    def forward(self, feat: Tensor, graph: Dict) -> Tensor:
        if _hot_guard(feat, *ops.module_params(self)):
            return lane_conv_train(self.fuse, feat, lane_plan(graph), lane_plan_t(graph), len(graph["pre"]),
                                   fused_bwd=M2M.train_hip)
        return ops.guarded(lambda: lane_conv(self.fuse, feat, lane_plan(graph), len(graph["pre"])))


def build_pairs(agt_idcs, agt_ctrs, ctx_idcs, ctx_ctrs, dist_th, legacy_offsets=True) -> ops.PairSet:
    ta = [int(len(x)) for x in agt_idcs]
    tc = [int(len(x)) for x in ctx_idcs]
    dev = agt_ctrs[0].device
    off = np.zeros((2, len(ta) + 1), np.int32)
    np.cumsum(ta, out=off[0, 1:])
    np.cumsum(tc, out=off[1, 1:])
    off_d = torch.from_numpy(off).to(dev)
    cap = int(np.dot(np.asarray(ta, np.int64), np.asarray(tc, np.int64)))
    return ops.pairs_build(torch.cat(agt_ctrs, 0), off_d[0], torch.cat(ctx_ctrs, 0), off_d[1],
                           dist_th, cap, legacy_offsets)


class Att(nn.Module):
    strict = True
    legacy_offsets = True
    fold = True
    train_hip = False

    def __init__(self, n_agt: int, n_ctx: int) -> None:
        super().__init__()
        self.dist = nn.Sequential(nn.Linear(2, n_ctx), nn.ReLU(inplace=True),
                                  Linear(n_ctx, n_ctx, norm="GN", ng=1))
        self.query = Linear(n_agt, n_ctx, norm="GN", ng=1)
        self.ctx = nn.Sequential(Linear(3 * n_ctx, n_agt, norm="GN", ng=1), nn.Linear(n_agt, n_agt, bias=False))
        self.agt = nn.Linear(n_agt, n_agt, bias=False)
        self.norm = nn.GroupNorm(gcd(1, n_agt), n_agt)
        self.linear = Linear(n_agt, n_agt, norm="GN", ng=1, act=False)
        self.relu = nn.ReLU(inplace=True)

    def forward(self, agts: Tensor, agt_idcs: List[Tensor], agt_ctrs: List[Tensor], ctx: Tensor,
                ctx_idcs: List[Tensor], ctx_ctrs: List[Tensor], dist_th: float,
                pairs: Optional[ops.PairSet] = None) -> Tensor:
        train = _hot_guard(agts, ctx, *ops.module_params(self))
        T = agts.shape[0]
        lin = self.linear
        if len(ctx) == 0:
            if train:
                a = A.linear_gn(agts, self.agt.weight, relu=True)
                return A.linear_gn(a, lin.linear.weight, gn=lin.norm, relu=True, res=agts)
            return ops.guarded(lambda: ops.agg_mlp(T, [ops.RelSpec(agts, ops.packed(self.agt.weight))],
                                                   L.F_RELU1 | L.F_GEMM2 | L.F_GN2 | L.F_RES | L.F_RELU2,
                                                   wp2=ops.packed(lin.linear.weight), gn2=_gn(lin.norm), res=agts,
                                                   eps=lin.norm.eps))
        ps = pairs if pairs is not None else build_pairs(agt_idcs, agt_ctrs, ctx_idcs, ctx_ctrs, dist_th,
                                                         self.legacy_offsets)
        if (self.strict or train) and ps.count() == 0:
            raise RuntimeError("torch.cat(): expected a non-empty list of Tensors")
        return self.run_train(agts, ctx, ps) if train else ops.guarded(lambda: self.run(agts, ctx, ps))

    def _train_hip_ok(self, agts: Tensor, ctx: Tensor, ps: ops.PairSet) -> bool:
# ... 697 lines not shown
```

lanegcn-1_amd/ops.py:

```python
import ctypes as C
from dataclasses import dataclass
from typing import List, Optional, Sequence, Tuple

import torch

from . import _lib as L

import os

C_FEAT = 128
EPS = 1e-5

_mma = L.MMA_NAMES[os.environ.get("LGCN_MMA", "f16x2")]


def set_mma(name: str):
    global _mma
    _mma = L.MMA_NAMES[name]


def get_mma() -> str:
    return {v: k for k, v in L.MMA_NAMES.items()}[_mma]


# ... 165 lines not shown
                raise L.LgcnError("pair capacity %d exceeded (P = %d)" % (self.cap, -self._p_host))
        return self._p_host

    def csr_by_wi(self, n_ctx: int):
        if getattr(self, "_wcsr", None) is None:
            P = self.count()
            wi = self.wi[:P].long()
            order = torch.argsort(wi, stable=True)
            counts = torch.zeros(n_ctx, dtype=torch.int64, device=wi.device).index_add_(0, wi, torch.ones_like(wi))
            rowptr = torch.zeros(n_ctx + 1, dtype=torch.int32, device=wi.device)
            rowptr[1:] = torch.cumsum(counts, 0).to(torch.int32)
            self._wcsr = (rowptr, order.to(torch.int32).contiguous())
        return self._wcsr

    def hi_wi_long(self):
        lib = L.load()
        P = self.count()
        h = torch.empty(self.cap, dtype=torch.int64, device=self.hi.device)
        w = torch.empty_like(h)
        L.check(lib.lgcn_widen_i32(_ptr(self.hi), _ptr(self.n_pairs), self.cap, _ptr(h), _stream()), "lgcn_widen_i32")
        L.check(lib.lgcn_widen_i32(_ptr(self.wi), _ptr(self.n_pairs), self.cap, _ptr(w), _stream()), "lgcn_widen_i32")
        return h[:P], w[:P]


def pairs_alloc(n_agt: int, n_scenes: int, cap: int, device):
    lib = L.load()
    i32 = dict(dtype=torch.int32, device=device)
    return (torch.empty(max(cap, 1), **i32), torch.empty(max(cap, 1), **i32), torch.empty(1, **i32),
            torch.empty(n_agt + 1, **i32), torch.empty(lib.lgcn_pairs_ws_elems(n_agt, n_scenes), **i32))


def pairs_build(agt_ctrs: torch.Tensor, agt_off: torch.Tensor, ctx_ctrs: torch.Tensor, ctx_off: torch.Tensor,
                dist_th: float, cap: int, legacy_offsets: bool = True, bufs=None) -> PairSet:
    lib = L.load()
    agt_ctrs = _dev(agt_ctrs, torch.float32, "agt_ctrs")
    ctx_ctrs = _dev(ctx_ctrs, torch.float32, "ctx_ctrs")
    agt_off = _dev(agt_off, torch.int32, "agt_off")
    ctx_off = _dev(ctx_off, torch.int32, "ctx_off")
    B = agt_off.numel() - 1
    if ctx_off.numel() != B + 1 or B < 1:
        raise L.LgcnError("pairs_build: offset tables must both have B+1 entries")
    T, S = agt_ctrs.shape[0], ctx_ctrs.shape[0]
    hi, wi, n_pairs, rowptr, ws = bufs if bufs is not None else pairs_alloc(T, B, cap, agt_ctrs.device)
    L.check(lib.lgcn_pairs_build(_ptr(agt_ctrs), _ptr(agt_off), _ptr(ctx_ctrs), _ptr(ctx_off), B, T, S,
                                 float(dist_th), int(bool(legacy_offsets)), _ptr(hi), _ptr(wi), cap,
                                 _ptr(n_pairs), _ptr(rowptr), _ptr(ws), _stream()), "lgcn_pairs_build")
    return PairSet(hi, wi, n_pairs, rowptr, cap, T, agt_ctrs, ctx_ctrs)


def pairs_build_multi(searches, legacy_offsets: bool = True, bufs=None) -> List["PairSet"]:
    lib = L.load()
    n = len(searches)
    if n < 1 or n > 4:
        raise L.LgcnError("pairs_build_multi: 1..4 searches")
    jobs, out, keep = _pairs_jobs(searches, legacy_offsets, bufs)
    L.check(lib.lgcn_pairs_build_multi(jobs, n, _stream()), "lgcn_pairs_build_multi")
    return out


def _pairs_jobs(searches, legacy_offsets, bufs):
    n = len(searches)
    jobs = (L.PairsJob * max(n, 1))()
    out, keep = [], []
    for k, (agt_ctrs, agt_off, ctx_ctrs, ctx_off, dist_th, cap) in enumerate(searches):
        agt_ctrs = _dev(agt_ctrs, torch.float32, "agt_ctrs")
        ctx_ctrs = _dev(ctx_ctrs, torch.float32, "ctx_ctrs")
        agt_off = _dev(agt_off, torch.int32, "agt_off")
        ctx_off = _dev(ctx_off, torch.int32, "ctx_off")
        B = agt_off.numel() - 1
        if ctx_off.numel() != B + 1 or B < 1:
            raise L.LgcnError("pair search: offset tables must both have B+1 entries")
        T, S = agt_ctrs.shape[0], ctx_ctrs.shape[0]
        hi, wi, n_pairs, rowptr, ws = bufs[k] if bufs is not None else pairs_alloc(T, B, cap, agt_ctrs.device)
        j = jobs[k]
        j.agt_ctrs, j.agt_off, j.ctx_ctrs, j.ctx_off = agt_ctrs.data_ptr(), agt_off.data_ptr(), ctx_ctrs.data_ptr(), ctx_off.data_ptr()
        j.n_scenes, j.legacy_offsets, j.n_agt, j.n_ctx, j.dist_th = B, int(bool(legacy_offsets)), T, S, float(dist_th)
        j.hi, j.wi, j.cap = hi.data_ptr(), wi.data_ptr(), cap
        j.n_pairs, j.rowptr, j.ws = n_pairs.data_ptr(), rowptr.data_ptr(), ws.data_ptr()
        keep += [agt_ctrs, ctx_ctrs, agt_off, ctx_off, ws]
        out.append(PairSet(hi, wi, n_pairs, rowptr, cap, T, agt_ctrs, ctx_ctrs))
    return jobs, out, keep


def index_counters(n_nodes: int, n_rel: int, device) -> torch.Tensor:
    lib = L.load()
    return torch.zeros(lib.lgcn_index_cnt_words(n_nodes, n_rel), dtype=torch.int64, device=device)


def index_fused_ok(n_nodes: int, n_rel: int, n_edges_total: int) -> bool:
    lib = L.load()
    return n_edges_total < (1 << 31) and lib.lgcn_csr_rowptr_elems(n_nodes, n_rel) <= (1 << 22)


def index_build(idx_local: torch.Tensor, seg_off: torch.Tensor, seg_base: torch.Tensor, rel_slices, n_nodes: int,
                searches=(), legacy_offsets: bool = True, bufs=None, cnt: Optional[torch.Tensor] = None,
                clear_word: Optional[torch.Tensor] = None):
    lib = L.load()
    idx_local = _dev(idx_local, torch.int64, "idx_local")
    seg_off = _dev(seg_off, torch.int64, "seg_off")
    seg_base = _dev(seg_base, torch.int64, "seg_base")
    n_rel = len(rel_slices)
    if n_rel < 1 or n_rel > L.MAX_REL or len(searches) > 4:
        raise L.LgcnError("index_build: 1..%d relations, <= 4 pair searches" % L.MAX_REL)
    dev = idx_local.device
    ne = [int(ub - ua) for (ua, ub), _ in rel_slices]
    nk1 = lib.lgcn_csr_rowptr_elems(n_nodes, n_rel)
    rowptr = torch.empty(nk1, dtype=torch.int32, device=dev)
    col = torch.empty(max(sum(ne), 1), dtype=torch.int32, device=dev)
    uv = torch.empty(max(2 * sum(ne), 2), dtype=torch.int32, device=dev)
    if cnt is None:
        cnt = index_counters(n_nodes, n_rel, dev)
    elif cnt.numel() < lib.lgcn_index_cnt_words(n_nodes, n_rel) or cnt.dtype != torch.int64 or cnt.device != dev:
        raise L.LgcnError("index_build: counter buffer of the wrong size / type / device")
    jobs, pairs, keep = _pairs_jobs(searches, legacy_offsets, bufs)
    p = L.Index()
    p.idx_local, p.n_elem = idx_local.data_ptr(), idx_local.numel()
    p.seg_off, p.seg_base, p.n_seg, p.n_rel = seg_off.data_ptr(), seg_base.data_ptr(), seg_base.numel(), n_rel
    for r, ((ua, ub), (va, vb)) in enumerate(rel_slices):
        if vb - va != ub - ua:
            raise L.LgcnError("index_build: u and v runs differ in length")
        p.u_off[r], p.v_off[r], p.n_edges[r] = ua, va, ub - ua
    p.n_nodes = n_nodes
    p.rowptr, p.col, p.cnt, p.uv = rowptr.data_ptr(), col.data_ptr(), cnt.data_ptr(), uv.data_ptr()
    p.jobs, p.n_jobs = C.cast(jobs, C.c_void_p).value if len(searches) else 0, len(searches)
    p.clear_word = 0 if clear_word is None else _dev(clear_word, torch.int32, "clear_word").data_ptr()
    L.check(lib.lgcn_index_build(C.byref(p), _stream()), "lgcn_index_build")
    plan = LanePlan(rowptr, col, n_rel, n_nodes, ne)
    plan.__dict__["_idx_keep"] = (cnt, uv, keep)
    return plan, pairs


def conv_packed(weight: torch.Tensor) -> torch.Tensor:
    def make():
        lib = L.load()
        cout, cin, ks = weight.shape
        nbytes = lib.lgcn_conv_packed_bytes(cin, cout, ks)
        if nbytes < 0:
            raise L.LgcnError("conv_packed: unsupported Conv1d weight shape %s" % (tuple(weight.shape),))
        out = torch.empty(nbytes // 4, dtype=torch.int32, device=weight.device)
        w = _dev(weight.detach(), torch.float32, "weight")
        L.check(lib.lgcn_conv_pack_weight(_ptr(w), cin, cout, ks, _ptr(out), _stream()), "lgcn_conv_pack_weight")
        return out
    return _cached(weight, ("conv",), make)


def conv_packed_f32(weight: torch.Tensor) -> torch.Tensor:
    def make():
        lib = L.load()
        cout, cin, ks = weight.shape
        nbytes = lib.lgcn_conv_packed_f32_bytes(cin, cout, ks)
        if nbytes < 0:
            raise L.LgcnError("conv_packed_f32: unsupported Conv1d weight shape %s" % (tuple(weight.shape),))
        out = torch.empty(nbytes // 4, dtype=torch.float32, device=weight.device)
        w = _dev(weight.detach(), torch.float32, "weight")
        L.check(lib.lgcn_conv_pack_weight_f32(_ptr(w), cin, cout, ks, _ptr(out), _stream()), "lgcn_conv_pack_weight_f32")
        return out
    return _cached(weight, ("convF32",), make)


def conv1d_gn(x: torch.Tensor, weight: torch.Tensor, stride: int, gamma, beta, eps: float, res: Optional[torch.Tensor] = None,
              res_up2: bool = False, relu: bool = False, exact: bool = False) -> torch.Tensor:
    lib = L.load()
    x = _dev(x, torch.float32, "x")
    A_, lin, cin = x.shape
    cout, cin_w, ks = weight.shape
    if cin_w != cin:
        raise L.LgcnError("conv1d_gn: weight does not match the input's channels")
    lout = (lin + 2 * ((ks - 1) // 2) - ks) // stride + 1
    out = torch.empty((A_, lout, cout), dtype=torch.float32, device=x.device)
    mode = 0
    if res is not None:
        res = _dev(res, torch.float32, "res")
        mode = 2 if res_up2 else 1
        if tuple(res.shape) != ((A_, lout // 2, cout) if res_up2 else (A_, lout, cout)):
            raise L.LgcnError("conv1d_gn: residual of the wrong shape")
    if exact:
        L.check(lib.lgcn_conv1d_gn_f32(_ptr(x), A_, lin, cin, _ptr(conv_packed_f32(weight)), cout, ks, stride,
                                       _ptr(_dev(gamma.detach(), torch.float32, "gamma")),
                                       _ptr(_dev(beta.detach(), torch.float32, "beta")), float(eps), _ptr(res), mode,
                                       int(bool(relu)), _ptr(out), None, _stream()), "lgcn_conv1d_gn_f32")
        return out
    L.check(lib.lgcn_conv1d_gn(_ptr(x), A_, lin, cin, _ptr(conv_packed(weight)), cout, ks, stride,
                               _ptr(_dev(gamma.detach(), torch.float32, "gamma")), _ptr(_dev(beta.detach(), torch.float32, "beta")),
                               float(eps), _ptr(res), mode, int(bool(relu)), _ptr(out), _stream()), "lgcn_conv1d_gn")
    return out


def conv_packed_t(weight: torch.Tensor) -> torch.Tensor:
    def make():
        lib = L.load()
        cout, cin, ks = weight.shape
        nbytes = lib.lgcn_conv_packed_t_bytes(cin, cout, ks)
        if nbytes < 0:
            raise L.LgcnError("conv_packed_t: unsupported Conv1d weight shape %s" % (tuple(weight.shape),))
        out = torch.empty(nbytes // 4, dtype=torch.float32, device=weight.device)
        w = _dev(weight.detach(), torch.float32, "weight")
        L.check(lib.lgcn_conv_pack_weight_t(_ptr(w), cin, cout, ks, _ptr(out), _stream()), "lgcn_conv_pack_weight_t")
        return out
    return _cached(weight, ("convT",), make)


def conv1d_gn_train(x: torch.Tensor, weight: torch.Tensor, stride: int, gamma, beta, eps: float,
                    res: Optional[torch.Tensor] = None, res_up2: bool = False, relu: bool = False, exact: bool = False):
    lib = L.load()
    x = _dev(x, torch.float32, "x")
    A_, lin, cin = x.shape
    cout, cin_w, ks = weight.shape
    if cin_w != cin:
        raise L.LgcnError("conv1d_gn_train: weight does not match the input's channels")
# ... 1454 lines not shown
```

Before: 139,200 scenes/s.

## Add two-launch per-run CSR index build with fused MapNet stem tiles

Adds a new index build path that counts edges per 64-node run in one launch and then builds each run's CSR rows and columns in block-local LDS in a second launch. The lane-pair count search and the MapNet input stem GEMM tiles are folded into the same first launch, so the stem no longer needs its own kernel. This is meant to cut kernel launches and the global sort/scan passes of the older multi-kernel index build. In exchange it adds a large amount of new code guarded by size limits on scenes, rows and edges, and it falls back to the old path when inputs do not fit those limits.

```diff
diff --git a/include/lgcn.h b/include/lgcn.h
--- a/include/lgcn.h
+++ b/include/lgcn.h
@@ -67,6 +67,21 @@
 int64_t lgcn_index_uv_elems(int64_t n_edges);
 int64_t lgcn_index_cnt_words(int64_t n_nodes, int n_rel);
 int lgcn_index_build(const lgcn_index_t *p_host, void *stream);
+
+typedef struct {
+    const int32_t *node_off; int32_t n_scenes, pad_;
+    int32_t *ctr;
+    int32_t *pair_cnt;
+    const float *ctrs, *feats; int64_t stem_n_rows;
+    const float *wa1, *ba1, *wpa2, *ga, *bta;
+    const float *ws1, *bs1, *wps2, *gs, *bts;
+    float stem_eps; int32_t stem_mma;
+    float *stem_out;
+} lgcn_index2_t;
+int64_t lgcn_index2_cnt_words(void);
+int64_t lgcn_index2_pair_ws_elems(int64_t n_agt);
+int lgcn_index2_ok(int64_t n_nodes, int n_rel, int n_scenes, int64_t max_scene_edges, int64_t max_scene_rows);
+int lgcn_index_build2(const lgcn_index_t *p_host, const lgcn_index2_t *x_host, void *stream);
 
 
 int64_t lgcn_conv_packed_bytes(int cin, int cout, int ks);
diff --git a/lanegcn-1_amd/_lib.py b/lanegcn-1_amd/_lib.py
--- a/lanegcn-1_amd/_lib.py
+++ b/lanegcn-1_amd/_lib.py
@@ -38,6 +38,18 @@
         ("rowptr", C.c_void_p), ("col", C.c_void_p), ("cnt", C.c_void_p), ("uv", C.c_void_p),
         ("jobs", C.c_void_p), ("n_jobs", C.c_int32), ("pad_", C.c_int32),
         ("clear_word", C.c_void_p),
+    ]
+
+
+class Index2(C.Structure):
+    _fields_ = [
+        ("node_off", C.c_void_p), ("n_scenes", C.c_int32), ("pad_", C.c_int32),
+        ("ctr", C.c_void_p), ("pair_cnt", C.c_void_p),
+        ("ctrs", C.c_void_p), ("feats", C.c_void_p), ("stem_n_rows", C.c_int64),
+        ("wa1", C.c_void_p), ("ba1", C.c_void_p), ("wpa2", C.c_void_p), ("ga", C.c_void_p), ("bta", C.c_void_p),
+        ("ws1", C.c_void_p), ("bs1", C.c_void_p), ("wps2", C.c_void_p), ("gs", C.c_void_p), ("bts", C.c_void_p),
+        ("stem_eps", C.c_float), ("stem_mma", C.c_int32),
+        ("stem_out", C.c_void_p),
     ]
 
 
@@ -234,6 +246,10 @@
     "lgcn_index_uv_elems": (C.c_int64, [_L]),
     "lgcn_index_cnt_words": (C.c_int64, [_L, _I]),
     "lgcn_index_build": (C.c_int, [_P, _P]),
+    "lgcn_index2_cnt_words": (C.c_int64, []),
+    "lgcn_index2_pair_ws_elems": (C.c_int64, [_L]),
+    "lgcn_index2_ok": (C.c_int, [_L, _I, _I, _L, _L]),
+    "lgcn_index_build2": (C.c_int, [_P, _P, _P]),
     "lgcn_att_pairs_ws": (C.c_int, [_P, _P, _P, _P, _P, _L] + [_P] * 10 + [_F, _I, _I, _P, _P]),
     "lgcn_att_pairs_wi": (C.c_int, [_P, _P, _P, _P, _P, _L] + [_P] * 10 + [_F, _I, _I, _P, _P]),
     "lgcn_pack_weight_kperm": (C.c_int, [_P, _I, _I, _P, _P]),
diff --git a/lanegcn-1_amd/csrc/lgcn_index.hip b/lanegcn-1_amd/csrc/lgcn_index.hip
--- a/lanegcn-1_amd/csrc/lgcn_index.hip
+++ b/lanegcn-1_amd/csrc/lgcn_index.hip
@@ -1,4 +1,6 @@
 #include "lgcn_common.hpp"
+#include "lgcn_tile.hpp"
+#include "lgcn_mma_bf.hpp"
 
 namespace lgcn {
 
@@ -335,12 +337,13 @@
     PairsJobs jobs;
 };
 
-__device__ __forceinline__ int64_t to_global(const IndexParams &p, int64_t i) {
+__device__ __forceinline__ int64_t to_global(const IndexParams &p, int64_t i, int *seg = nullptr) {
     int lo = 0, hi = p.n_seg;
     while (hi - lo > 1) {
         const int mid = (lo + hi) >> 1;
         if (p.seg_off[mid] <= i) lo = mid; else hi = mid;
     }
+    if (seg) *seg = lo;
     return p.idx_local[i] + p.seg_base[lo];
 }
 
@@ -436,6 +439,432 @@
         while (q >= 0 && c[q] > x) { c[q + 1] = c[q]; --q; }
         c[q + 1] = x;
     }
+}
+
+constexpr int kRunNodes = 64;
+constexpr int kMaxRuns = 1024;
+constexpr int kRunKeysMax = kRunNodes * LGCN_MAX_REL;
+constexpr int kRunColCap = 4096;
+constexpr int kRunSegMax = 256;
+constexpr int kIdx2MaxScenes = 1023;
+constexpr int kIdx2MaxRows = 65536;
+constexpr int kIdx2Ctr = kMaxRuns + 2;
+constexpr int64_t kIdx2MaxSceneEdges = 16384;
+constexpr int64_t kIdx2MaxSceneRows = 4096;
+
+struct Index2Params {
+    IndexParams p;
+    const int32_t *node_off;
+    int n_scenes, n_runs, stem_tiles;
+    int32_t *ctr;
+    int32_t *pair_cnt;
+    int job_ws0[4];
+    InputParams stem;
+};
+__device__ __forceinline__ int32_t *idx2_flag(const Index2Params &q) { return q.ctr + kMaxRuns; }
+
+__device__ __forceinline__ int wave_sum(int v) {
+#pragma unroll
+    for (int off = 32; off >= 1; off >>= 1) v += __shfl_xor(v, off, 64);
+    return v;
+}
+
+__device__ __forceinline__ void idx2_pairs_count(const PairsJob &j, int32_t *ws, int block, int *lds) {
+    const int lane = threadIdx.x & 63, wave = threadIdx.x >> 6;
+    const int g0 = 16 * block + 4 * wave;
+    const int sc0 = g0 < j.n_agt ? find_scene(j.agt_off, j.n_scenes, g0) : 0;
+    const int end0 = g0 < j.n_agt ? j.agt_off[sc0 + 1] : 0;
+    int wsum = 0;
+#pragma unroll
+    for (int i = 0; i < 4; ++i) {
+        const int g = g0 + i;
+        if (g < j.n_agt) {
+            const int sc = g < end0 || sc0 + 1 >= j.n_scenes ? sc0 : find_scene(j.agt_off, j.n_scenes, g);
+            int c0 = j.ctx_off[sc], c1 = j.ctx_off[sc + 1];
+            c0 = c0 < 0 ? 0 : c0 > j.n_ctx ? j.n_ctx : c0;
+            c1 = c1 < c0 ? c0 : c1 > j.n_ctx ? j.n_ctx : c1;
+            const float2 a = j.agt[g];
+            int count = 0;
+            for (int s0 = c0; s0 < c1; s0 += 64) {
+                const int s = s0 + lane;
+                bool ok = false;
+                if (s < c1) {
+                    const float2 c = j.ctx[s];
+                    ok = within(a.x, a.y, c.x, c.y, j.th);
+                }
+                count += __popcll(__ballot(ok));
+            }
+            if (lane == 0) ws[g] = count;
+            wsum += count;
+        }
+    }
+    if (lane == 0) lds[wave] = wsum;
+    __syncthreads();
+    if (threadIdx.x == 0) ws[j.n_agt + block] = lds[0] + lds[1] + lds[2] + lds[3];
+}
+
+template <int RB, int F>
+struct StemSmem { static constexpr int BYTES = Tile<RB, F>::ABUF_BYTES + Tile<RB, F>::T_BYTES; };
+template <int F>
+struct StemSmem<0, F> { static constexpr int BYTES = 0; };
+
+template <int RB, int F>
+__global__ __launch_bounds__(256) void k_index2_count(const Index2Params q) {
+    constexpr int SMEM = StemSmem<RB, F>::BYTES > kMaxRuns * 4 ? StemSmem<RB, F>::BYTES : kMaxRuns * 4;
+    __shared__ __attribute__((aligned(16))) unsigned char smem[SMEM];
+    const IndexParams &p = q.p;
+    if (blockIdx.x == 0 && threadIdx.x == 0 && p.clear_word) *p.clear_word = 0;
+    int bid = blockIdx.x;
+    if (bid < q.stem_tiles) {
+        if constexpr (RB > 0) mapnet_input_body<RB, F>(q.stem, bid, smem);
+        return;
+    }
+    bid -= q.stem_tiles;
+    if (bid >= p.edge_blocks) {
+        const int b = bid - p.edge_blocks;
+        int jn = 0;
+        while (jn + 1 < p.n_jobs && b >= p.job_blocks[jn + 1]) ++jn;
+        idx2_pairs_count(p.jobs.j[jn], q.pair_cnt + q.job_ws0[jn], b - p.job_blocks[jn], reinterpret_cast<int *>(smem));
+        return;
+    }
+    int *s_run = reinterpret_cast<int *>(smem);
+    for (int i = threadIdx.x; i < q.n_runs; i += blockDim.x) s_run[i] = 0;
+    __syncthreads();
+    const int B = q.n_scenes;
+    bool cross = false;
+    const int64_t total = p.start[p.n_rel];
+    for (int64_t e = (int64_t)bid * blockDim.x + threadIdx.x; e < total; e += (int64_t)p.edge_blocks * blockDim.x) {
+        int r = 0;
+        while (r + 1 < p.n_rel && e >= p.start[r + 1]) ++r;
+        const int64_t le = e - p.start[r];
+        int su, sv;
+        const int64_t u = to_global(p, p.u_off[r] + le, &su), v = to_global(p, p.v_off[r] + le, &sv);
+        const bool ok = u >= 0 && u < p.n_nodes && v >= 0 && v < p.n_nodes;
+        p.uv[2 * e] = ok ? (int32_t)u : -1;
+        p.uv[2 * e + 1] = (int32_t)v;
+        if (ok) {
+            atomicAdd(&s_run[u / kRunNodes], 1);
+            const int sc = su - r * 2 * B;
+            if (sc < 0 || sc >= B || u < q.node_off[sc] || u >= q.node_off[sc + 1]) cross = true;
+        }
+    }
+    if (cross) *idx2_flag(q) = 1;
+    __syncthreads();
+    for (int i = threadIdx.x; i < q.n_runs; i += blockDim.x)
+        if (s_run[i] != 0) atomicAdd(&q.ctr[i], s_run[i]);
+}
+
+constexpr int kB2 = 1024;
+
+struct Idx2RunLds {
+    int scan[kB2 / 64 + 1];
+    int off[kRunKeysMax + 1];
+    int cur[kRunKeysMax];
+    int col[kRunColCap];
+    int m[kRunColCap];
+    int noff[kIdx2MaxScenes + 1];
+    int seg_lo[kRunSegMax], seg_pre[kRunSegMax + 1], seg_e0[kRunSegMax];
+    int nm, s_lo, s_hi;
+};
+struct Idx2PairLds {
+    int scan[kB2 / 64 + 1];
+    int cpre[kIdx2MaxRows / 16 + 1];
+    int raw[kIdx2MaxScenes + 1];
+    int pre[kIdx2MaxScenes + 1];
+    int ctxn[kIdx2MaxScenes];
+};
+union Idx2Lds { Idx2RunLds run; Idx2PairLds pair; };
+
+__device__ __forceinline__ int find_scene_lds(const int *off, int n_scenes, int g) {
+    int lo = 0, hi = n_scenes;
+    while (hi - lo > 1) {
+        const int mid = (lo + hi) >> 1;
+        if (off[mid] <= g) lo = mid; else hi = mid;
+    }
+    return lo;
+}
+
+template <class Fn>
+__device__ __forceinline__ void run_candidates(const Index2Params &q, bool cross, int s_lo, int s_hi, int64_t n0, int64_t n1, Fn fn) {
+    const IndexParams &p = q.p;
+    const int2 *uv = reinterpret_cast<const int2 *>(p.uv);
+    if (cross) {
+        const int64_t total = p.start[p.n_rel];
+        for (int64_t e = threadIdx.x; e < total; e += blockDim.x) {
+            int r = 0;
+            while (r + 1 < p.n_rel && e >= p.start[r + 1]) ++r;
+            const int2 x = uv[e];
+            if (x.x >= n0 && x.x < n1) fn(r, x.x, x.y);
+        }
+        return;
+    }
+    const int B = q.n_scenes;
+    for (int r = 0; r < p.n_rel; ++r) {
+        const int64_t ne = p.start[r + 1] - p.start[r];
+        for (int s = s_lo; s <= s_hi; ++s) {
+            int64_t lo = p.seg_off[r * 2 * B + s] - p.u_off[r], hi = p.seg_off[r * 2 * B + s + 1] - p.u_off[r];
+            lo = lo < 0 ? 0 : lo > ne ? ne : lo;
+            hi = hi < lo ? lo : hi > ne ? ne : hi;
+            for (int64_t le = lo + threadIdx.x; le < hi; le += blockDim.x) {
+                const int2 x = uv[p.start[r] + le];
+                if (x.x >= n0 && x.x < n1) fn(r, x.x, x.y);
+            }
+        }
+    }
+}
+
+__device__ __forceinline__ void sort_keys(int *c, int n) {
+    for (int a = 1; a < n; ++a) {
+        const int x = c[a];
+        int j = a - 1;
+        while (j >= 0 && c[j] > x) { c[j + 1] = c[j]; --j; }
+        c[j + 1] = x;
+    }
+}
+
+__device__ __forceinline__ void idx2_run_build(const Index2Params &q, int run, Idx2RunLds &s) {
+    const IndexParams &p = q.p;
+    const int tid = threadIdx.x, lane = tid & 63, n_rel = p.n_rel, B = q.n_scenes;
+    const int64_t npad = (p.n_nodes + 15) / 16 * 16;
+    const int64_t n0 = (int64_t)run * kRunNodes;
+    const int64_t n1 = n0 + kRunNodes < npad ? n0 + kRunNodes : npad;
+    const int K = (int)(n1 - n0) * n_rel;
+    const int64_t k0 = n0 * n_rel;
+    const int64_t total = p.start[n_rel];
+    const int2 *uv = reinterpret_cast<const int2 *>(p.uv);
+    const int part = tid < run ? q.ctr[tid] : 0;
+    const bool cross = *idx2_flag(q) != 0;
+    if (tid <= B) s.noff[tid] = q.node_off[tid];
+    if (tid < K) { s.off[tid] = 0; s.cur[tid] = 0; }
+    if (tid == 0) s.nm = 0;
+    int base;
+    block_exclusive_scan<kB2>(part, &base, s.scan);
+    const int64_t last = (n1 < p.n_nodes ? n1 : p.n_nodes) - 1;
+    const bool any = last >= n0;
+    const int s_lo = any ? find_scene_lds(s.noff, B, (int)n0) : 0, s_hi = any ? find_scene_lds(s.noff, B, (int)last) : -1;
+    const int n_seg = (s_hi - s_lo + 1) * n_rel;
+    const bool listed = !cross && n_seg <= kRunSegMax;
+    bool stashed = false;
+    if (listed) {
+        int len = 0;
+        if (tid < n_seg) {
+            const int r = tid / (s_hi - s_lo + 1), sc = s_lo + tid % (s_hi - s_lo + 1);
+            const int64_t ne = p.start[r + 1] - p.start[r];
+            int64_t lo = p.seg_off[r * 2 * B + sc] - p.u_off[r], hi = p.seg_off[r * 2 * B + sc + 1] - p.u_off[r];
+            lo = lo < 0 ? 0 : lo > ne ? ne : lo;
+            hi = hi < lo ? lo : hi > ne ? ne : hi;
+            len = (int)(hi - lo);
+            s.seg_e0[tid] = (int)(p.start[r] + lo);
+        }
+        int C;
+        const int pre = block_exclusive_scan<kB2>(len, &C, s.scan);
+        if (tid < n_seg) s.seg_pre[tid] = pre;
+        if (tid == 0) s.seg_pre[n_seg] = C;
+        __syncthreads();
+        for (int c0 = 0; c0 < C; c0 += 4 * kB2) {
+            int2 x[4];
+            int sg[4];
+#pragma unroll
+            for (int k = 0; k < 4; ++k) {
+                const int c = c0 + k * kB2 + tid;
+                sg[k] = c < C ? find_scene_lds(s.seg_pre, n_seg, c) : 0;
+                x[k] = c < C ? uv[s.seg_e0[sg[k]] + (c - s.seg_pre[sg[k]])] : make_int2(-1, 0);
+            }
+#pragma unroll
+            for (int k = 0; k < 4; ++k) {
+                const bool hit = x[k].x >= n0 && x[k].x < n1;
+                const int word = hit ? (int)(csr_key(x[k].x, sg[k] / (s_hi - s_lo + 1), n_rel) - k0) << 16 | x[k].y : 0;
+                const unsigned long long mk = __ballot(hit);
+                if (mk != 0ull) {
+                    int w0 = 0;
+                    if (lane == 0) w0 = atomicAdd(&s.nm, __popcll(mk));
+                    w0 = __shfl(w0, 0, 64);
+                    const int slot = w0 + __popcll(mk & ((1ull << lane) - 1ull));
+                    if (hit && slot < kRunColCap) s.m[slot] = word;
+                }
+            }
+        }
+        __syncthreads();
+        stashed = s.nm <= kRunColCap;
+    }
+    if (stashed) {
+        const int nm = s.nm;
+        for (int i = tid; i < nm; i += kB2) atomicAdd(&s.off[s.m[i] >> 16], 1);
+    } else {
+        run_candidates(q, cross, s_lo, s_hi, n0, n1, [&](int r, int u, int) { atomicAdd(&s.off[(int)(csr_key(u, r, n_rel) - k0)], 1); });
+    }
+    __syncthreads();
+    const int cntk = tid < K ? s.off[tid] : 0;
+    int T;
+    const int off = block_exclusive_scan<kB2>(cntk, &T, s.scan);
+    if (tid < K) s.off[tid] = off;
+    if (tid == 0) s.off[K] = T;
+    __syncthreads();
+    if (tid < K) p.rowptr[k0 + tid] = base + off;
+    if (run == q.n_runs - 1 && tid == 0) p.rowptr[k0 + K] = base + T;
+    if (stashed) {
+        for (int i = tid; i < T; i += kB2) {
+            const int w = s.m[i], kl = w >> 16;
+            s.col[s.off[kl] + atomicAdd(&s.cur[kl], 1)] = w & 0xffff;
+        }
+        __syncthreads();
+        if (tid < K) sort_keys(s.col + off, cntk);
+        __syncthreads();
+        for (int i = tid; i < T; i += kB2)
+            if (base + i < total) p.col[base + i] = s.col[i];
+    } else {
+        run_candidates(q, cross, s_lo, s_hi, n0, n1, [&](int r, int u, int vv) {
+            const int kl = (int)(csr_key(u, r, n_rel) - k0);
+            const int pos = s.off[kl] + atomicAdd(&s.cur[kl], 1);
+            if (base + pos < total) p.col[base + pos] = vv;
+        });
+        __syncthreads();
+        if (tid < K) {
+            int n = cntk;
+            if ((int64_t)base + off + n > total) n = (int64_t)base + off < total ? (int)(total - base - off) : 0;
+            sort_keys(p.col + base + off, n);
+        }
+    }
+}
+
+__device__ __forceinline__ void idx2_pair_tables(const PairsJob &j, const int32_t *ws, Idx2PairLds &s) {
+    const int tid = threadIdx.x, B = j.n_scenes;
+    const int n_blocks = (j.n_agt + 15) / 16;
+    const int32_t *bsum = ws + j.n_agt;
+    int raw = 0;
+    if (tid <= B) raw = j.agt_off[tid];
+    if (tid < B) s.ctxn[tid] = j.ctx_off[tid + 1] - j.ctx_off[tid];
+    int carry = 0;
+    for (int c0 = 0; c0 < n_blocks; c0 += kB2) {
+        const int c = c0 + tid;
+        const int v = c < n_blocks ? bsum[c] : 0;
+        int tot;
+        const int pre = block_exclusive_scan<kB2>(v, &tot, s.scan);
+        if (c < n_blocks) s.cpre[c] = pre + carry;
+        carry += tot;
+    }
+    if (tid == 0) s.cpre[n_blocks] = carry;
+    __syncthreads();
+    if (tid <= B) {
+        const int a = raw < 0 ? 0 : raw > j.n_agt ? j.n_agt : raw;
+        int pre = s.cpre[a >> 4];
+#pragma unroll
+        for (int k = 0; k < 15; ++k) pre += (a & ~15) + k < a ? ws[(a & ~15) + k] : 0;
+        s.raw[tid] = raw;
+        s.pre[tid] = pre;
+    }
+    __syncthreads();
+}
+
+__device__ __forceinline__ void idx2_scene_terms(const PairsJob &j, const Idx2PairLds &s, int i, int *t, int *th, int *tw) {
+    int a0 = s.raw[i], a1 = s.raw[i + 1];
+    a0 = a0 < 0 ? 0 : a0 > j.n_agt ? j.n_agt : a0;
+    a1 = a1 < a0 ? a0 : a1 > j.n_agt ? j.n_agt : a1;
+    *t = a1 > a0 ? s.pre[i + 1] - s.pre[i] : 0;
+    const bool adv = !j.legacy || *t > 0;
+    *th = adv ? a1 - a0 : 0;
+    *tw = adv ? s.ctxn[i] : 0;
+}
+
+__device__ __forceinline__ void idx2_job_header(const PairsJob &j, const int32_t *ws, Idx2PairLds &s) {
+    idx2_pair_tables(j, ws, s);
+    const int tid = threadIdx.x;
+    int t = 0, th = 0, tw = 0;
+    if (tid < j.n_scenes) idx2_scene_terms(j, s, tid, &t, &th, &tw);
+    int tot_h, tot_w;
+    const int ph = block_exclusive_scan<kB2>(th, &tot_h, s.scan);
+    const int pw = block_exclusive_scan<kB2>(tw, &tot_w, s.scan);
+    if (tid < j.n_scenes) { j.hi_base()[tid] = ph; j.wi_base()[tid] = pw; }
+    if (tid == 0) {
+        const int P = s.cpre[(j.n_agt + 15) / 16];
+        j.hi_base()[j.n_scenes] = tot_h;
+        j.rp()[j.n_agt] = P;
+        *j.n_pairs = (int64_t)P > j.cap ? -P : P;
+        if (j.n_agt == 0) j.rowptr_q[0] = 0;
+    }
+}
+
+__device__ __forceinline__ void idx2_pairs_fill(const PairsJob &j, const int32_t *ws, int block, Idx2PairLds &s) {
+    idx2_pair_tables(j, ws, s);
+    const int lane = threadIdx.x & 63;
+    const int g = 16 * block + (threadIdx.x >> 6);
+    const int n_agt = j.n_agt, n_scenes = j.n_scenes;
+    if (g >= n_agt) return;
+    const int sc = find_scene_lds(s.raw, n_scenes, g);
+    int c0 = j.ctx_off[sc], c1 = j.ctx_off[sc + 1];
+    c0 = c0 < 0 ? 0 : c0 > j.n_ctx ? j.n_ctx : c0;
+    c1 = c1 < c0 ? c0 : c1 > j.n_ctx ? j.n_ctx : c1;
+    const float2 a = j.agt[g];
+    const int beside = lane < (g & 15) ? ws[(g & ~15) + lane] : 0;
+    int hb = 0, wb = 0, h_used = 0, t_sc = 0;
+    for (int s0 = 0; s0 < n_scenes; s0 += 64) {
+        const int i = s0 + lane;
+        if (i < n_scenes) {
+            int t, th, tw;
+            idx2_scene_terms(j, s, i, &t, &th, &tw);
+            if (i < sc) { hb += th; wb += tw; }
+            if (i == sc) t_sc = t;
+            h_used += th;
+        }
+    }
+    hb = wave_sum(hb); wb = wave_sum(wb); h_used = wave_sum(h_used); t_sc = wave_sum(t_sc);
+    int64_t pos = s.cpre[g >> 4] + wave_sum(beside);
+    const int P = s.cpre[(n_agt + 15) / 16];
+    const int hval = g - s.raw[sc] + hb, wbase = wb - c0;
+    if (lane == 0) {
+        j.rp()[g] = (int)pos;
+        const bool advances = !j.legacy || t_sc > 0;
+        const int q2 = h_used + g - hb;
+        const int Pc = (int64_t)P > j.cap ? (int)j.cap : P;
+        if (advances) { if (hval >= 0 && hval <= n_agt) j.rowptr_q[hval] = pos > j.cap ? (int)j.cap : (int)pos; }
+        else if (q2 >= 0 && q2 <= n_agt) j.rowptr_q[q2] = Pc;
+        if (g == 0) j.rowptr_q[n_agt] = Pc;
+    }
+    for (int s0 = c0; s0 < c1; s0 += 64) {
+        const int sx = s0 + lane;
+        bool ok = false;
+        if (sx < c1) {
+            const float2 c = j.ctx[sx];
+            ok = within(a.x, a.y, c.x, c.y, j.th);
+        }
+        const unsigned long long m = __ballot(ok);
+        if (ok) {
+            const int64_t o = pos + __popcll(m & ((1ull << lane) - 1ull));
+            if (o < j.cap) { j.hi[o] = hval; j.wi[o] = sx + wbase; }
+        }
+        pos += __popcll(m);
+    }
+}
+
+__global__ __launch_bounds__(kB2) void k_index2_build(const Index2Params q) {
+    __shared__ Idx2Lds s;
+    __shared__ int s_last;
+    const IndexParams &p = q.p;
+    const int bid = blockIdx.x;
+    if (bid >= q.n_runs) {
+        if (bid < q.n_runs + p.n_jobs) {
+            const int jn = bid - q.n_runs;
+            idx2_job_header(p.jobs.j[jn], q.pair_cnt + q.job_ws0[jn], s.pair);
+        } else {
+            const int b = bid - q.n_runs - p.n_jobs;
+            int jn = 0;
+            while (jn + 1 < p.n_jobs && b >= p.job_blocks[jn + 1]) ++jn;
+            idx2_pairs_fill(p.jobs.j[jn], q.pair_cnt + q.job_ws0[jn], b - p.job_blocks[jn], s.pair);
+        }
+        return;
+    }
+    idx2_run_build(q, bid, s.run);
+    asm volatile("s_waitcnt vmcnt(0) lgkmcnt(0)" ::: "memory");
+    __syncthreads();
+    if (threadIdx.x == 0) s_last = atomicAdd(&q.ctr[kIdx2Ctr - 1], 1) == q.n_runs - 1;
+    __syncthreads();
+    if (s_last)
+        for (int i = threadIdx.x; i < kIdx2Ctr; i += kB2) q.ctr[i] = 0;
+}
+
+template <int RB, int F>
+static void launch_index2_count(unsigned grid, hipStream_t st, const Index2Params &d) {
+    hipLaunchKernelGGL((k_index2_count<RB, F>), dim3(grid), dim3(256), 0, st, d);
 }
 
 __global__ __launch_bounds__(256) void k_sq_bound(const int32_t *rowptr, const int32_t *col, int64_t n, int32_t *ub) {
@@ -705,15 +1134,13 @@
     return k < 0 ? k : k + kIdxMaxTiles;
 }
 
-int lgcn_index_build(const lgcn_index_t *ph, void *stream) {
-    LGCN_CHECK_PTR(ph);
-    const lgcn_index_t &q = *ph;
+static int index_params(const lgcn_index_t &q, bool need_cnt, IndexParams &p, int64_t *total_out) {
     if (q.n_rel < 1 || q.n_rel > LGCN_MAX_REL || q.n_nodes < 0 || q.n_seg < 1 || q.n_jobs < 0 || q.n_jobs > 4 || q.n_elem < 0)
         return LGCN_EINVAL;
-    LGCN_CHECK_PTR(q.rowptr); LGCN_CHECK_PTR(q.cnt);
+    LGCN_CHECK_PTR(q.rowptr);
+    if (need_cnt) LGCN_CHECK_PTR(q.cnt);
     if (((uintptr_t)q.cnt & 7u) != 0) return LGCN_EALIGN;
     if (q.n_jobs > 0) LGCN_CHECK_PTR(q.jobs);
-    IndexParams p;
     p.idx_local = q.idx_local; p.seg_off = q.seg_off; p.seg_base = q.seg_base; p.n_seg = q.n_seg; p.n_rel = q.n_rel;
     p.start[0] = 0;
     for (int r = 0; r < q.n_rel; ++r) {
@@ -758,6 +1185,18 @@
         for (int k = 0; k < 4; ++k) p.jobs.j[k] = z;
     }
     p.edge_blocks = total > 0 ? (int)grid_for(total, 256, 1024) : 0;
+    *total_out = total;
+    return LGCN_OK;
+}
+
+int lgcn_index_build(const lgcn_index_t *ph, void *stream) {
+    LGCN_CHECK_PTR(ph);
+    const lgcn_index_t &q = *ph;
+    IndexParams p;
+    int64_t total;
+    const int rc = index_params(q, true, p, &total);
+    if (rc != LGCN_OK) return rc;
+    const int64_t nk1 = p.n_keys1;
     p.scan_blocks = (int)((nk1 + kIdxScanTile - 1) / kIdxScanTile);
     hipStream_t st = (hipStream_t)stream;
     const unsigned g13 = (unsigned)(p.edge_blocks + p.job_blocks[4]);
@@ -766,6 +1205,90 @@
     hipLaunchKernelGGL(k_index_scan, dim3((unsigned)(p.scan_blocks + q.n_jobs)), dim3(1024), 0, st, p);
     if (g13 > 0) hipLaunchKernelGGL((k_index_edges<1>), dim3(g13), dim3(256), 0, st, p);
     if (total > 0) hipLaunchKernelGGL(k_index_sort, dim3((unsigned)((nk1 + 255) / 256)), dim3(256), 0, st, p);
+    return launch_status();
+}
+
+int64_t lgcn_index2_cnt_words(void) { return (kIdx2Ctr + 1) / 2; }
+
+int64_t lgcn_index2_pair_ws_elems(int64_t n_agt) { return n_agt < 0 ? (int64_t)LGCN_EINVAL : n_agt + (n_agt + 15) / 16; }
+
+int lgcn_index2_ok(int64_t n_nodes, int n_rel, int n_scenes, int64_t max_scene_edges, int64_t max_scene_rows) {
+    return n_nodes >= 0 && n_nodes < (int64_t)kMaxRuns * kRunNodes && n_rel >= 1 && n_rel <= LGCN_MAX_REL && n_scenes >= 1 &&
+           n_scenes <= kIdx2MaxScenes && max_scene_edges >= 0 && max_scene_edges <= kIdx2MaxSceneEdges && max_scene_rows >= 0 &&
+           max_scene_rows <= kIdx2MaxSceneRows;
+}
+
+int lgcn_index_build2(const lgcn_index_t *ph, const lgcn_index2_t *xh, void *stream) {
+    LGCN_CHECK_PTR(ph); LGCN_CHECK_PTR(xh);
+    const lgcn_index_t &q = *ph;
+    const lgcn_index2_t &x = *xh;
+    Index2Params d;
+    int64_t total;
+    int rc = index_params(q, false, d.p, &total);
+    if (rc != LGCN_OK) return rc;
+    d.p.scan_blocks = 0;
+    if (x.n_scenes < 1 || x.n_scenes > kIdx2MaxScenes) return LGCN_EINVAL;
+    if (q.n_nodes >= (int64_t)kMaxRuns * kRunNodes) return LGCN_ESHAPE;
+    if ((int64_t)q.n_seg != 2 * (int64_t)q.n_rel * x.n_scenes) return LGCN_EINVAL;
+    LGCN_CHECK_PTR(x.node_off); LGCN_CHECK_PTR(x.ctr); LGCN_CHECK_PTR(q.seg_off);
+    if (((uintptr_t)q.uv & 7u) != 0) return LGCN_EALIGN;
+    int64_t ws = 0;
+    d.p.job_blocks[0] = 0;
+    for (int k = 0; k < 4; ++k) {
+        d.job_ws0[k] = (int)ws;
+        d.p.job_blocks[k + 1] = d.p.job_blocks[k];
+        if (k < q.n_jobs) {
+            if (q.jobs[k].n_scenes > kIdx2MaxScenes || q.jobs[k].n_agt > kIdx2MaxRows) return LGCN_ESHAPE;
+            ws += lgcn_index2_pair_ws_elems(q.jobs[k].n_agt);
+            d.p.job_blocks[k + 1] += (int)((q.jobs[k].n_agt + 15) / 16);
+        }
+    }
+    if (ws > 0) LGCN_CHECK_PTR(x.pair_cnt);
+    d.node_off = x.node_off; d.n_scenes = x.n_scenes;
+    d.n_runs = (int)((q.n_nodes + kRunNodes - 1) / kRunNodes);
+    if (d.n_runs < 1) d.n_runs = 1;
+    d.ctr = x.ctr; d.pair_cnt = x.pair_cnt;
+    d.stem_tiles = 0;
+    d.stem = InputParams{};
+    int rb = 0, fmt = 0;
+    if (x.stem_n_rows > 0) {
+        if (x.stem_mma != LGCN_MMA_BF16X3 && x.stem_mma != LGCN_MMA_BF16 && x.stem_mma != LGCN_MMA_F16X2) return LGCN_EINVAL;
+        if (x.stem_n_rows > 0x7fffffff) return LGCN_ESHAPE;
+        const void *ptrs[] = {x.ctrs, x.feats, x.wa1, x.ba1, x.wpa2, x.ga, x.bta, x.ws1, x.bs1, x.wps2, x.gs, x.bts, x.stem_out};
+        for (const void *pp : ptrs) LGCN_CHECK_PTR(pp);
+        const void *al[] = {x.wa1, x.ba1, x.wpa2, x.ga, x.bta, x.ws1, x.bs1, x.wps2, x.gs, x.bts, x.stem_out};
+        for (const void *pp : al) LGCN_CHECK_ALIGN16(pp);
+        d.stem = InputParams{x.ctrs, x.feats, x.stem_n_rows, x.wa1, x.ba1, x.wpa2, x.ga, x.bta, x.ws1, x.bs1, x.wps2, x.gs, x.bts,
+                             x.stem_eps, x.stem_out};
+        rb = mapnet_input_rb(x.stem_n_rows, x.stem_mma);
+        fmt = fmt_of(x.stem_mma);
+        d.stem_tiles = (int)((x.stem_n_rows + 16 * rb - 1) / (16 * rb));
+    } else if (x.stem_n_rows < 0) {
+        return LGCN_EINVAL;
+    }
+    hipStream_t st = (hipStream_t)stream;
+    const unsigned ga = (unsigned)(d.stem_tiles + d.p.edge_blocks + d.p.job_blocks[4]);
+    if (ga == 0) {
+        if (q.clear_word) { hipError_t e = hipMemsetAsync(q.clear_word, 0, 4, st); if (e != hipSuccess) return (int)e; }
+    } else {
+        switch (rb * 4 + fmt) {
+            case 0: launch_index2_count<0, 0>(ga, st, d); break;
+            case 4: launch_index2_count<1, 0>(ga, st, d); break;
+            case 5: launch_index2_count<1, 1>(ga, st, d); break;
+            case 6: launch_index2_count<1, 2>(ga, st, d); break;
+            case 8: launch_index2_count<2, 0>(ga, st, d); break;
+            case 9: launch_index2_count<2, 1>(ga, st, d); break;
+            case 10: launch_index2_count<2, 2>(ga, st, d); break;
+            case 12: launch_index2_count<3, 0>(ga, st, d); break;
+            case 13: launch_index2_count<3, 1>(ga, st, d); break;
+            case 14: launch_index2_count<3, 2>(ga, st, d); break;
+            case 16: launch_index2_count<4, 0>(ga, st, d); break;
+            case 17: launch_index2_count<4, 1>(ga, st, d); break;
+            case 18: launch_index2_count<4, 2>(ga, st, d); break;
+            default: return LGCN_EINVAL;
+        }
+    }
+    hipLaunchKernelGGL(k_index2_build, dim3((unsigned)(d.n_runs + q.n_jobs + d.p.job_blocks[4])), dim3(kB2), 0, st, d);
     return launch_status();
 }
 
diff --git a/lanegcn-1_amd/csrc/lgcn_mma_bf.hpp b/lanegcn-1_amd/csrc/lgcn_mma_bf.hpp
--- a/lanegcn-1_amd/csrc/lgcn_mma_bf.hpp
+++ b/lanegcn-1_amd/csrc/lgcn_mma_bf.hpp
@@ -233,4 +233,58 @@
 }
 
 
-}
+template <int RB, int F>
+__device__ __forceinline__ void mapnet_input_body(const InputParams &p, int tile, unsigned char *smem) {
+    using TL = Tile<RB, F>;
+    constexpr int ROWS = TL::ROWS;
+    uint16_t *A = reinterpret_cast<uint16_t *>(smem);
+    float *T = reinterpret_cast<float *>(smem + TL::ABUF_BYTES);
+    const int tid = threadIdx.x, lane = tid & 63, wave = tid >> 6;
+    const int64_t row0 = (int64_t)tile * ROWS;
+    f32x4 acc[RB][2];
+    RowVals keep[(ROWS + 31) / 32];
+
+#pragma unroll
+    for (int br = 0; br < 2; ++br) {
+        const float2 *xy = reinterpret_cast<const float2 *>(br == 0 ? p.ctrs : p.feats);
+        const float *w1 = br == 0 ? p.wa1 : p.ws1, *b1 = br == 0 ? p.ba1 : p.bs1;
+        const float *wp = br == 0 ? p.wpa2 : p.wps2;
+        const float *g = br == 0 ? p.ga : p.gs, *bt = br == 0 ? p.bta : p.bts;
+#pragma unroll
+        for (int c0 = 0; c0 < ROWS; c0 += 32) {
+            const int row = c0 + (tid >> 3);
+            if (row < ROWS) {
+                float2 v = make_float2(0.f, 0.f);
+                if (row0 + row < p.n_rows) v = xy[row0 + row];
+                lin2_relu_split<F>(A, TL::PLANE, row, tid, v.x, v.y, w1, b1);
+            }
+        }
+        lds_barrier();
+        acc_zero<RB>(acc);
+        {
+            BPair<F> bf;
+            ring_prime<F>(bf, reinterpret_cast<const uint4 *>(wp), wave, lane);
+            gemm_pass<RB, F>(A, reinterpret_cast<const uint4 *>(wp), nullptr, bf, wave, lane, acc);
+        }
+        acc_store<RB>(T, acc, lane, wave);
+        lds_barrier();
+#pragma unroll
+        for (int c0 = 0; c0 < ROWS; c0 += 32) {
+            const int row = c0 + (tid >> 3);
+            if (row < ROWS) {
+                RowVals r = row_load(T + c0 * kLDA, tid);
+                row_gn<F == 0>(r, tid, g, bt, p.eps);
+                if (br == 0) {
+                    keep[c0 / 32] = r;
+                } else {
+#pragma unroll
+                    for (int j = 0; j < 4; ++j) r.v[j] = f4add(r.v[j], keep[c0 / 32].v[j]);
+                    row_relu(r);
+                    if (row0 + row < p.n_rows) row_store_global(p.out + (row0 + row) * kC, tid, r);
+                }
+            }
+        }
+    }
+}
+
+}
diff --git a/lanegcn-1_amd/csrc/lgcn_rowmlp_bf.hip b/lanegcn-1_amd/csrc/lgcn_rowmlp_bf.hip
--- a/lanegcn-1_amd/csrc/lgcn_rowmlp_bf.hip
+++ b/lanegcn-1_amd/csrc/lgcn_rowmlp_bf.hip
@@ -482,57 +482,8 @@
 
 template <int RB, int F>
 __global__ __launch_bounds__(256) void k_mapnet_input_bf(const InputParams p, int n_tiles) {
-    using TL = Tile<RB, F>;
-    constexpr int ROWS = TL::ROWS;
-    __shared__ __attribute__((aligned(16))) unsigned char smem[TL::ABUF_BYTES + TL::T_BYTES];
-    uint16_t *A = reinterpret_cast<uint16_t *>(smem);
-    float *T = reinterpret_cast<float *>(smem + TL::ABUF_BYTES);
-    const int tid = threadIdx.x, lane = tid & 63, wave = tid >> 6;
-    const int64_t row0 = (int64_t)blockIdx.x * ROWS;
-    f32x4 acc[RB][2];
-    RowVals keep[(ROWS + 31) / 32];
-
-#pragma unroll
-    for (int br = 0; br < 2; ++br) {
-        const float2 *xy = reinterpret_cast<const float2 *>(br == 0 ? p.ctrs : p.feats);
-        const float *w1 = br == 0 ? p.wa1 : p.ws1, *b1 = br == 0 ? p.ba1 : p.bs1;
-        const float *wp = br == 0 ? p.wpa2 : p.wps2;
-        const float *g = br == 0 ? p.ga : p.gs, *bt = br == 0 ? p.bta : p.bts;
-#pragma unroll
-        for (int c0 = 0; c0 < ROWS; c0 += 32) {
-            const int row = c0 + (tid >> 3);
-            if (row < ROWS) {
-                float2 v = make_float2(0.f, 0.f);
-                if (row0 + row < p.n_rows) v = xy[row0 + row];
-                lin2_relu_split<F>(A, TL::PLANE, row, tid, v.x, v.y, w1, b1);
-            }
-        }
-        lds_barrier();
-        acc_zero<RB>(acc);
-        {
-            BPair<F> bf;
-            ring_prime<F>(bf, reinterpret_cast<const uint4 *>(wp), wave, lane);
-            gemm_pass<RB, F>(A, reinterpret_cast<const uint4 *>(wp), nullptr, bf, wave, lane, acc);
-        }
-        acc_store<RB>(T, acc, lane, wave);
-        lds_barrier();
-#pragma unroll
-        for (int c0 = 0; c0 < ROWS; c0 += 32) {
-            const int row = c0 + (tid >> 3);
-            if (row < ROWS) {
-                RowVals r = row_load(T + c0 * kLDA, tid);
-                row_gn<F == 0>(r, tid, g, bt, p.eps);
-                if (br == 0) {
-                    keep[c0 / 32] = r;
-                } else {
-#pragma unroll
-                    for (int j = 0; j < 4; ++j) r.v[j] = f4add(r.v[j], keep[c0 / 32].v[j]);
-                    row_relu(r);
-                    if (row0 + row < p.n_rows) row_store_global(p.out + (row0 + row) * kC, tid, r);
-                }
-            }
-        }
-    }
+    __shared__ __attribute__((aligned(16))) unsigned char smem[Tile<RB, F>::ABUF_BYTES + Tile<RB, F>::T_BYTES];
+    mapnet_input_body<RB, F>(p, (int)blockIdx.x, smem);
 }
 
 static int cu_count() {
@@ -620,8 +571,10 @@
     });
 }
 
+int mapnet_input_rb(int64_t n_rows, int mma) { return pick_rb(n_rows, fmt_of(mma)); }
+
 int mapnet_input_bf(const InputParams &p, int mma, hipStream_t st) {
-    const int rb = pick_rb(p.n_rows, fmt_of(mma));
+    const int rb = mapnet_input_rb(p.n_rows, mma);
     const int n_tiles = (int)((p.n_rows + 16 * rb - 1) / (16 * rb));
     return with_fmt_rb(mma, rb, [&](auto f, auto r) {
         hipLaunchKernelGGL((k_mapnet_input_bf<decltype(r)::value, decltype(f)::value>), dim3(n_tiles), dim3(256), 0, st, p, n_tiles);
diff --git a/lanegcn-1_amd/csrc/lgcn_tile.hpp b/lanegcn-1_amd/csrc/lgcn_tile.hpp
--- a/lanegcn-1_amd/csrc/lgcn_tile.hpp
+++ b/lanegcn-1_amd/csrc/lgcn_tile.hpp
@@ -215,6 +215,7 @@
 int agg_mlp_pair_bf(const lgcn_agg_mlp_t &a, const lgcn_agg_mlp_t &b, hipStream_t st);
 int agg_mlp_multi_bf(const lgcn_agg_mlp_t *const *ps, int n, hipStream_t st);
 int mapnet_input_bf(const InputParams &p, int mma, hipStream_t st);
+int mapnet_input_rb(int64_t n_rows, int mma);
 int pack_weight_bf(const float *W, int ld, int mma, int transpose, void *out, hipStream_t st);
 int pack_weight_batch_bf(const lgcn_pack_job_t *jobs, int n_jobs, int mma, hipStream_t st);
 
diff --git a/lanegcn-1_amd/engine.py b/lanegcn-1_amd/engine.py
--- a/lanegcn-1_amd/engine.py
+++ b/lanegcn-1_amd/engine.py
@@ -32,6 +32,12 @@
     cap_a2a: int
     n_edges: List[int]
     _buf: Optional[torch.Tensor] = None
+    max_scene_edges: Optional[int] = None
+    max_scene_rows: Optional[int] = None
+
+    def index_two_launch(self) -> bool:
+        return ops.index_two_launch_ok(self.n_nodes, len(self.rel_slices), self.n_scenes, self.seg_base.numel(),
+                                       self.max_scene_edges, self.max_scene_rows)
 
     def buf_view(self) -> Optional[torch.Tensor]:
         return self._buf
@@ -74,6 +80,7 @@
     np.cumsum(n_act, out=actor_off[1:])
 
     pieces, seg_len, seg_base, rel_slices, n_edges = [], [], [], [], []
+    scene_len = np.zeros(B, np.int64)
     pos = 0
 
     def add(getter):
@@ -83,6 +90,7 @@
             x = npy(getter(g)).astype(np.int64, copy=False).reshape(-1)
             pieces.append(x)
             seg_len.append(len(x))
+            scene_len[j] += len(x)
             seg_base.append(node_off[j])
             pos += len(x)
         return (begin, pos)
@@ -126,7 +134,8 @@
         view[o:o + a.nbytes] = a.view(np.uint8).reshape(-1)
     meta = dict(n_scenes=B, n_nodes=int(node_off[-1]), n_actors=int(actor_off[-1]), num_scales=ns,
                 rel_slices=rel_slices, cap_a2m=int(np.dot(n_nodes, n_act)), cap_a2a=int(np.dot(n_act, n_act)),
-                n_edges=n_edges)
+                n_edges=n_edges, max_scene_edges=int(scene_len.max() // 2) if B else 0,
+                max_scene_rows=int(max(n_nodes.max(), n_act.max())) if B else 0)
     return HostFlatBatch(buf, layout, meta)
 
 
@@ -163,9 +172,18 @@
             return self._cnt_capture
         cnt = fb.__dict__.get("_idx_cnt")
         if cnt is None:
-            cnt = ops.index_counters(fb.n_nodes, len(fb.rel_slices), fb.node_ctrs.device)
+            cnt = self._new_counters(fb)
             fb.__dict__["_idx_cnt"] = cnt
         return cnt
+
+    @staticmethod
+    def _new_counters(fb: FlatBatch) -> torch.Tensor:
+        return ops.index_counters(fb.n_nodes, len(fb.rel_slices), fb.node_ctrs.device,
+                                  two_launch=fb.index_two_launch())
+
+    @staticmethod
+    def _index_kw(fb: FlatBatch) -> Dict:
+        return dict(node_off=fb.node_off, max_scene_edges=fb.max_scene_edges, max_scene_rows=fb.max_scene_rows)
 
     @torch.no_grad()
     def forward(self, fb: FlatBatch, actors: torch.Tensor, stages: bool = False,
@@ -196,8 +214,11 @@
             side.wait_stream(main)
         if side is None and ops.index_fused_ok(fb.n_nodes, len(fb.rel_slices), sum(fb.n_edges)):
             flag = torch.empty(1, dtype=torch.int32, device=dev)
+            stem = self.map_net.stem_job(fb.node_ctrs, fb.node_feats)
             plan, pairs = ops.index_build(fb.idx_local, fb.seg_off, fb.seg_base, fb.rel_slices, fb.n_nodes, searches,
-                                          self.legacy_offsets, bufs=bufs, cnt=self._counters(fb), clear_word=flag)
+                                          self.legacy_offsets, bufs=bufs, cnt=self._counters(fb), clear_word=flag,
+                                          stem=stem, **self._index_kw(fb))
+            feat = stem.out
         else:
             flag = torch.zeros(1, dtype=torch.int32, device=dev)
             with torch.cuda.stream(side if side is not None else main):
@@ -206,7 +227,7 @@
             us = [g64[a:b] for (a, b), _ in fb.rel_slices]
             vs = [g64[a:b] for _, (a, b) in fb.rel_slices]
             plan = ops.csr_build(us, vs, fb.n_nodes)
-        feat = self.map_net.stem(fb.node_ctrs, fb.node_feats)
+            feat = self.map_net.stem(fb.node_ctrs, fb.node_feats)
         feat = M.lane_conv(self.map_net.fuse, feat, plan, fb.num_scales, impl=self.lane_impl)
         if stages:
             out["map_net"] = feat
@@ -281,18 +302,21 @@
             if ops.index_fused_ok(fb.n_nodes, len(fb.rel_slices), sum(fb.n_edges)):
                 cnt = st.get("_cnt")
                 if cnt is None:
-                    cnt = st["_cnt"] = ops.index_counters(fb.n_nodes, len(fb.rel_slices), fb.node_ctrs.device)
+                    cnt = st["_cnt"] = self._new_counters(fb)
+                stem = self.map_net.stem_job(fb.node_ctrs, fb.node_feats)
                 st["plan"], st["pairs"] = ops.index_build(fb.idx_local, fb.seg_off, fb.seg_base, fb.rel_slices, fb.n_nodes,
-                                                          searches, self.legacy_offsets, cnt=cnt)
+                                                          searches, self.legacy_offsets, cnt=cnt, stem=stem,
+                                                          **self._index_kw(fb))
+                st["stem"] = stem.out
                 return
+            st["stem"] = self.map_net.stem(fb.node_ctrs, fb.node_feats)
             st["pairs"] = ops.pairs_build_multi(searches, self.legacy_offsets)
             g64, _ = ops.graph_gather_indices(fb.idx_local, fb.seg_off, fb.seg_base)
             st["plan"] = ops.csr_build([g64[a:b] for (a, b), _ in fb.rel_slices],
                                        [g64[a:b] for _, (a, b) in fb.rel_slices], fb.n_nodes)
 
         def map_net():
-            st["nodes"] = M.lane_conv(self.map_net.fuse, self.map_net.stem(fb.node_ctrs, fb.node_feats), st["plan"],
-                                      fb.num_scales, impl=self.lane_impl)
+            st["nodes"] = M.lane_conv(self.map_net.fuse, st["stem"], st["plan"], fb.num_scales, impl=self.lane_impl)
 
         def a2m():
             st["nodes_a2m"] = self.a2m.run(st["nodes"], fb.turn, fb.control, fb.intersect, actors, st["pairs"][0])
@@ -343,7 +367,7 @@
 
         @contextlib.contextmanager
         def cm():
-            cnt = ops.index_counters(fb.n_nodes, len(fb.rel_slices), fb.node_ctrs.device)
+            cnt = self._new_counters(fb)
             torch.cuda.synchronize()
             prev, self._cnt_capture = self._cnt_capture, cnt
             try:
diff --git a/lanegcn-1_amd/flatfile.py b/lanegcn-1_amd/flatfile.py
--- a/lanegcn-1_amd/flatfile.py
+++ b/lanegcn-1_amd/flatfile.py
@@ -106,7 +106,9 @@
             node_off=up(node_off.astype(np.int32)), actor_off=up(actor_off.astype(np.int32)),
             idx_local=up(np.concatenate(pieces) if pieces else np.zeros(0, np.int64)), seg_off=up(seg_off),
             seg_base=up(np.asarray(seg_base, np.int64)), rel_slices=rel_slices,
-            cap_a2m=int(np.dot(n_nodes, n_act)), cap_a2a=int(np.dot(n_act, n_act)), n_edges=n_edges)
+            cap_a2m=int(np.dot(n_nodes, n_act)), cap_a2a=int(np.dot(n_act, n_act)), n_edges=n_edges,
+            max_scene_edges=max([int(sum(seg_len[j::len(idx)])) // 2 for j in range(len(idx))], default=0),
+            max_scene_rows=int(max(n_nodes.max(), n_act.max())) if len(idx) else 0)
         rep = np.repeat(np.asarray(idx), n_act)
         extras = {"actor_feats": up(a["actor_feats"][arow].transpose(0, 2, 1)), "rot": up(a["rot"][rep]),
                   "orig": up(a["orig"][rep]), "sizes": [int(x) for x in n_act]}
diff --git a/lanegcn-1_amd/lanegcn.py b/lanegcn-1_amd/lanegcn.py
--- a/lanegcn-1_amd/lanegcn.py
+++ b/lanegcn-1_amd/lanegcn.py
@@ -247,6 +247,13 @@
                                 a[0].weight, a[0].bias, ops.packed(a[2].linear.weight), _gn(a[2].norm),
                                 s[0].weight, s[0].bias, ops.packed(s[2].linear.weight), _gn(s[2].norm),
                                 eps=a[2].norm.eps)
+
+    def stem_job(self, ctrs: Tensor, feats: Tensor) -> "ops.StemJob":
+        a, s = self.input, self.seg
+        return ops.StemJob(ctrs, feats,
+                           a[0].weight, a[0].bias, ops.packed(a[2].linear.weight), _gn(a[2].norm),
+                           s[0].weight, s[0].bias, ops.packed(s[2].linear.weight), _gn(s[2].norm),
+                           eps=a[2].norm.eps)
 
     def forward(self, graph):
         if (len(graph["feats"]) == 0 or len(graph["pre"][-1]["u"]) == 0 or len(graph["suc"][-1]["u"]) == 0):
diff --git a/lanegcn-1_amd/ops.py b/lanegcn-1_amd/ops.py
--- a/lanegcn-1_amd/ops.py
+++ b/lanegcn-1_amd/ops.py
@@ -271,19 +271,38 @@
     return jobs, out, keep
 
 
-def index_counters(n_nodes: int, n_rel: int, device) -> torch.Tensor:
-    lib = L.load()
+def index_counters(n_nodes: int, n_rel: int, device, two_launch: bool = False) -> torch.Tensor:
+    lib = L.load()
+    if two_launch:
+        return torch.zeros(lib.lgcn_index2_cnt_words(), dtype=torch.int64, device=device)
     return torch.zeros(lib.lgcn_index_cnt_words(n_nodes, n_rel), dtype=torch.int64, device=device)
 
 
 def index_fused_ok(n_nodes: int, n_rel: int, n_edges_total: int) -> bool:
     lib = L.load()
     return n_edges_total < (1 << 31) and lib.lgcn_csr_rowptr_elems(n_nodes, n_rel) <= (1 << 22)
+
+
+def index_two_launch_ok(n_nodes: int, n_rel: int, n_scenes: int, n_seg: int, max_scene_edges: Optional[int],
+                        max_scene_rows: Optional[int]) -> bool:
+    if max_scene_edges is None or max_scene_rows is None or n_seg != 2 * n_rel * n_scenes:
+        return False
+    return bool(L.load().lgcn_index2_ok(n_nodes, n_rel, n_scenes, int(max_scene_edges), int(max_scene_rows)))
+
+
+class StemJob:
+
+    def __init__(self, ctrs, feats, wa1, ba1, wpa2, gn_a, ws1, bs1, wps2, gn_s, eps=EPS):
+        self.args = (ctrs, feats, wa1, ba1, wpa2, gn_a, ws1, bs1, wps2, gn_s)
+        self.eps = eps
+        self.out = None
 
 
 def index_build(idx_local: torch.Tensor, seg_off: torch.Tensor, seg_base: torch.Tensor, rel_slices, n_nodes: int,
                 searches=(), legacy_offsets: bool = True, bufs=None, cnt: Optional[torch.Tensor] = None,
-                clear_word: Optional[torch.Tensor] = None):
+                clear_word: Optional[torch.Tensor] = None, node_off: Optional[torch.Tensor] = None,
+                max_scene_edges: Optional[int] = None, max_scene_rows: Optional[int] = None,
+                stem: Optional[StemJob] = None):
     lib = L.load()
     idx_local = _dev(idx_local, torch.int64, "idx_local")
     seg_off = _dev(seg_off, torch.int64, "seg_off")
@@ -297,7 +316,17 @@
     rowptr = torch.empty(nk1, dtype=torch.int32, device=dev)
     col = torch.empty(max(sum(ne), 1), dtype=torch.int32, device=dev)
     uv = torch.empty(max(2 * sum(ne), 2), dtype=torch.int32, device=dev)
-    if cnt is None:
+    n_scenes = 0 if node_off is None else node_off.numel() - 1
+    two = (node_off is not None and seg_off.numel() > seg_base.numel() and
+           index_two_launch_ok(n_nodes, n_rel, n_scenes, seg_base.numel(), max_scene_edges, max_scene_rows) and
+           all(s[1].numel() - 1 <= 1023 and s[0].shape[0] <= 65536 for s in searches))
+    if two:
+        node_off = _dev(node_off, torch.int32, "node_off")
+        if cnt is None:
+            cnt = index_counters(n_nodes, n_rel, dev, two_launch=True)
+        elif cnt.numel() < lib.lgcn_index2_cnt_words() or cnt.dtype != torch.int64 or cnt.device != dev:
+            raise L.LgcnError("index_build: counter buffer of the wrong size / type / device")
+    elif cnt is None:
         cnt = index_counters(n_nodes, n_rel, dev)
     elif cnt.numel() < lib.lgcn_index_cnt_words(n_nodes, n_rel) or cnt.dtype != torch.int64 or cnt.device != dev:
         raise L.LgcnError("index_build: counter buffer of the wrong size / type / device")
@@ -313,7 +342,27 @@
     p.rowptr, p.col, p.cnt, p.uv = rowptr.data_ptr(), col.data_ptr(), cnt.data_ptr(), uv.data_ptr()
     p.jobs, p.n_jobs = C.cast(jobs, C.c_void_p).value if len(searches) else 0, len(searches)
     p.clear_word = 0 if clear_word is None else _dev(clear_word, torch.int32, "clear_word").data_ptr()
-    L.check(lib.lgcn_index_build(C.byref(p), _stream()), "lgcn_index_build")
+    if two:
+        x = L.Index2()
+        x.node_off, x.n_scenes, x.ctr = node_off.data_ptr(), n_scenes, cnt.data_ptr()
+        pair_cnt = torch.empty(max(sum(lib.lgcn_index2_pair_ws_elems(ps.n_agt) for ps in pairs), 1), dtype=torch.int32,
+                               device=dev)
+        x.pair_cnt = pair_cnt.data_ptr()
+        keep += [pair_cnt, node_off]
+        if stem is not None and _mma != L.MMA_F32 and stem.args[0].shape[0] > 0:
+            ctrs, feats, wa1, ba1, wpa2, gn_a, ws1, bs1, wps2, gn_s = stem.args
+            ctrs, feats = _dev(ctrs, torch.float32, "ctrs"), _dev(feats, torch.float32, "feats")
+            stem.out = torch.empty((ctrs.shape[0], C_FEAT), dtype=torch.float32, device=ctrs.device)
+            x.ctrs, x.feats, x.stem_n_rows = ctrs.data_ptr(), feats.data_ptr(), ctrs.shape[0]
+            x.wa1, x.ba1, x.wpa2, x.ga, x.bta = _ptr(wa1), _ptr(ba1), _ptr(wpa2), _ptr(gn_a[0]), _ptr(gn_a[1])
+            x.ws1, x.bs1, x.wps2, x.gs, x.bts = _ptr(ws1), _ptr(bs1), _ptr(wps2), _ptr(gn_s[0]), _ptr(gn_s[1])
+            x.stem_eps, x.stem_mma, x.stem_out = stem.eps, _mma, stem.out.data_ptr()
+            keep += [ctrs, feats]
+        L.check(lib.lgcn_index_build2(C.byref(p), C.byref(x), _stream()), "lgcn_index_build2")
+    else:
+        L.check(lib.lgcn_index_build(C.byref(p), _stream()), "lgcn_index_build")
+    if stem is not None and stem.out is None:
+        stem.out = mapnet_input(*stem.args, eps=stem.eps)
     plan = LanePlan(rowptr, col, n_rel, n_nodes, ne)
     plan.__dict__["_idx_keep"] = (cnt, uv, keep)
     return plan, pairs
```

Measured after the change: 137,500 scenes/s. 0.988x the previous value.
